# SamuelCancilla2/radar-point-cloud-tracking

Measured on AMD Instinct MI355X. Metric: Mpoints/s clustered+tracked, 1024-echo synthetic frames; 1/2/4/8-GPU scaling, higher is better.
Workload: dtype u8 echo / f32 geometry / f64 distance

## Files before the change

radar-point-cloud-tracking_amd/csrc/stdbscan.hip:

```cpp
#include <algorithm>
#include <cfloat>
#include <climits>
#include <cmath>
#include <cstdlib>
#include <cstring>
#include <mutex>
#include <vector>

#include "common.h"

#pragma clang fp contract(off)

namespace rpt {

namespace {

constexpr int kBlock = 256;

__device__ __forceinline__ uint32_t f2ord(float f) {
  uint32_t u = __float_as_uint(f);
  return (u & 0x80000000u) ? ~u : (u | 0x80000000u);
}
inline float ord2f(uint32_t u) {
  uint32_t v = (u & 0x80000000u) ? (u & 0x7fffffffu) : ~u;
// ... 173 lines not shown
    }
    sb[w].nonfinite_xyz = nonfin;
    sb[w].nonintegral_t = nonint;
    sb[w].n_finite_t = nfin;
    sb[w].t_descends = desc;
  }
  __syncthreads();
  if (threadIdx.x == 0) {
    for (int v = 1; v < kBlock / 64; ++v) {
      for (int k = 0; k < 4; ++k) {
        mn[k] = min(mn[k], sb[v].mn[k]);
        mx[k] = max(mx[k], sb[v].mx[k]);
      }
      nonfin |= sb[v].nonfinite_xyz;
      nonint |= sb[v].nonintegral_t;
      nfin += sb[v].n_finite_t;
      desc |= sb[v].t_descends;
    }
    for (int k = 0; k < 4; ++k) {
      out->mn[k] = mn[k];
      out->mx[k] = mx[k];
    }
    out->nonfinite_xyz = nonfin;
    out->nonintegral_t = nonint;
    out->n_finite_t = nfin;
    out->t_descends = desc;
  }
}

struct FastDiv {
  uint32_t m;
  int s;
  void init(uint32_t d) {
    int k = 0;
    while ((uint64_t(1) << k) < d) ++k;
    s = 31 + k;
    m = (uint32_t)(((uint64_t(1) << s) + d - 1) / d);
  }
  __device__ __forceinline__ uint32_t div(uint32_t n) const {
    return (uint32_t)(((uint64_t)n * m) >> s);
  }
};

struct Geom {
  double ox, oy, oz, ot;
  double cs;
  double ct;
  double inv_cs, inv_ct;
  int nx, ny, nz, nt;
  int64_t cells;
  double eps2;
  float epst;
  int min_samples;
  float e2lo, e2hi;
  int rt;
  int tfree;
  FastDiv fnx, fny, fnz, fslab;
  __device__ __forceinline__ void split(uint32_t k, int& x, int& y, int& z, int& s) const {
    const uint32_t r = fnx.div(k);
    x = (int)(k - r * (uint32_t)nx);
    const uint32_t r2 = fny.div(r);
    y = (int)(r - r2 * (uint32_t)ny);
    if (nz == 1) {
      z = 0;
      s = (int)r2;
    } else {
      const uint32_t r3 = fnz.div(r2);
      z = (int)(r2 - r3 * (uint32_t)nz);
      s = (int)r3;
    }
  }
  __device__ __forceinline__ int slab_of_key(int64_t k) const { return (int)fslab.div((uint32_t)k); }
};

__device__ __forceinline__ int cell_of(double v, double o, double inv, int n) {
  double q = floor((v - o) * inv);
  int c = (q < 0.0) ? 0 : (q >= (double)n ? n - 1 : (int)q);
  return c;
}
__device__ __forceinline__ int slab_of(float t, const Geom& g) {
  return cell_of((double)t, g.ot, g.inv_ct, g.nt);
}

template <int D>
__global__ __launch_bounds__(kBlock) void k_keys(const float* __restrict__ x,
                                                const float* __restrict__ y,
                                                const float* __restrict__ z, int64_t stride,
                                                const float* __restrict__ t, int64_t n, Geom g,
                                                uint32_t* __restrict__ keys,
                                                uint32_t* __restrict__ vals) {
  for (int64_t i = (int64_t)blockIdx.x * blockDim.x + threadIdx.x; i < n;
       i += (int64_t)gridDim.x * blockDim.x) {
    const float ti = t[i];
    uint32_t key;
    if (!isfinite(ti)) {
      key = (uint32_t)g.cells;
    } else {
      const int cx = cell_of((double)x[i * stride], g.ox, g.inv_cs, g.nx);
      const int cy = cell_of((double)y[i * stride], g.oy, g.inv_cs, g.ny);
      const int cz = (D == 3) ? cell_of((double)z[i * stride], g.oz, g.inv_cs, g.nz) : 0;
      const int s = slab_of(ti, g);
      key = (uint32_t)((((int64_t)s * g.nz + cz) * g.ny + cy) * g.nx + cx);
    }
    keys[i] = key;
    vals[i] = (uint32_t)i;
  }
}

template <int D>
__global__ __launch_bounds__(kBlock) void k_gather(const float* __restrict__ x,
                                                  const float* __restrict__ y,
                                                  const float* __restrict__ z, int64_t stride,
                                                  const float* __restrict__ t, int64_t n,
                                                  const uint32_t* __restrict__ skeys,
                                                  const uint32_t* __restrict__ svals,
                                                  float4* __restrict__ pts,
                                                  int32_t* __restrict__ sorig,
                                                  int32_t* __restrict__ skey,
                                                  int32_t* __restrict__ spos) {
  for (int64_t s = (int64_t)blockIdx.x * blockDim.x + threadIdx.x; s < n;
       s += (int64_t)gridDim.x * blockDim.x) {
    const int64_t i = svals[s];
    float4 p;
    p.x = x[i * stride];
    p.y = y[i * stride];
    p.w = t[i];
    p.z = (D == 3) ? z[i * stride] : p.w;
    pts[s] = p;
    sorig[s] = (int32_t)i;
    if (spos) spos[i] = (int32_t)s;
    skey[s] = (int32_t)skeys[s];
  }
}

__global__ __launch_bounds__(kBlock) void k_cell_runs(const int32_t* __restrict__ skey, int64_t n,
                                                     int32_t* __restrict__ cell_count,
                                                     int32_t* __restrict__ head) {
  for (int64_t s = (int64_t)blockIdx.x * blockDim.x + threadIdx.x; s < n;
       s += (int64_t)gridDim.x * blockDim.x) {
    const int32_t k = skey[s];
    const bool h = (s == 0) || skey[s - 1] != k;
    const bool t = (s == n - 1) || skey[s + 1] != k;
    if (h && t) {
      cell_count[k] = 1;
    } else {
      if (h) atomicAdd(cell_count + k, -(int32_t)s);
      if (t) atomicAdd(cell_count + k, (int32_t)(s + 1));
    }
    head[s] = h ? 1 : 0;
  }
}

__global__ __launch_bounds__(kBlock) void k_occ_list(const int32_t* __restrict__ skey, int64_t n,
                                                    const int32_t* __restrict__ pos,
                                                    int32_t* __restrict__ occ,
                                                    uint32_t* __restrict__ occ_bits) {
  for (int64_t s = (int64_t)blockIdx.x * blockDim.x + threadIdx.x; s < n;
       s += (int64_t)gridDim.x * blockDim.x)
    if (pos[s + 1] != pos[s]) {
      const int32_t c = skey[s];
      occ[pos[s]] = c;
      atomicOr(occ_bits + (c >> 5), 1u << (c & 31));
    }
}

constexpr int kBucketBlock = 1024;
// ... 2 lines not shown
constexpr int64_t kChunkPts = 16384;
static int slab_chunks_override() {
  static const int v = [] {
    const char* e = ab_env("RPT_SLAB_CHUNKS");
    return e ? std::atoi(e) : 0;
  }();
  return v;
}

static int ab_mode(const char* name) {
  const char* e = ab_env(name);
  const int v = e ? std::atoi(e) : 1;
  return (v == 0 || v == 2) ? v : 1;
}
static int cell_box_mixed() {
  static const int v = ab_mode("RPT_CELL_BOX_MIXED");
  return v;
}
static int union_snapshot() {
  static const int v = ab_mode("RPT_UNION_SNAP");
  return v;
}

static int label_core_orig() {
  static const int v = ab_mode("RPT_LABEL_ORIG");
  return v;
}

static bool cell_comp_enabled() {
  static const bool on = [] {
    const char* e = ab_env("RPT_CELL_COMP");
    return !(e && std::atoi(e) == 0);
  }();
  return on;
}

static bool chunk_scan_legacy() {
  static const bool v = [] {
    const char* e = ab_env("RPT_CHUNK_SCAN");
    return e && std::atoi(e) == 1;
  }();
  return v;
}

__global__ void k_slab_occ_base(const int32_t* __restrict__ pos, int P, int64_t nt,
                                int32_t* __restrict__ occ_base) {
  for (int64_t s = (int64_t)blockIdx.x * blockDim.x + threadIdx.x; s <= nt;
       s += (int64_t)gridDim.x * blockDim.x)
    occ_base[s] = pos[s * P];
}

__global__ void k_cell_start_end(int32_t* __restrict__ cell_start, int64_t cells) {
  if (threadIdx.x == 0) cell_start[cells + 1] = cell_start[cells];
}

__global__ void k_slab_lo(const float* __restrict__ t, int64_t n, Geom g,
                          int32_t* __restrict__ slab_lo, uint32_t* __restrict__ zero,
                          int64_t zwords) {
  for (int64_t i = (int64_t)blockIdx.x * blockDim.x + threadIdx.x; i < zwords;
       i += (int64_t)gridDim.x * blockDim.x)
    zero[i] = 0u;
  const int lane = threadIdx.x & 63;
  const int64_t wpb = blockDim.x / 64;
  for (int64_t s = (int64_t)blockIdx.x * wpb + threadIdx.x / 64; s <= g.nt;
       s += (int64_t)gridDim.x * wpb) {
    int64_t lo = 0, hi = n;
    while (lo < hi) {
      const int64_t step = (hi - lo + 63) / 64;
      const int64_t idx = lo + (int64_t)lane * step;
      const bool below = idx < hi && slab_of(t[idx < hi ? idx : lo], g) < s;
      const int c = __popcll(__ballot(below));
      if (c == 0) {
        hi = lo;
      } else {
        const int64_t nlo = lo + (int64_t)(c - 1) * step + 1;
        hi = min(hi, lo + (int64_t)c * step);
        lo = nlo;
      }
    }
    if (lane == 0) slab_lo[s] = (int32_t)(s == g.nt ? n : lo);
  }
}

__global__ __launch_bounds__(kBucketBlock) void k_slab_bucket(
    const float* __restrict__ x, const float* __restrict__ y, int64_t stride,
    const float* __restrict__ t, Geom g, const int32_t* __restrict__ slab_lo,
    float4* __restrict__ pts, int32_t* __restrict__ sorig, int32_t* __restrict__ skey,
    int32_t* __restrict__ spos, int32_t* __restrict__ cell_start, int32_t* __restrict__ occ_tmp,
    int32_t* __restrict__ slab_occ, uint32_t* __restrict__ occ_bits,
    unsigned long long* __restrict__ cmin_all = nullptr) {
  extern __shared__ int32_t hist[];
  __shared__ int32_t wsum[kBucketBlock / 64], wocc[kBucketBlock / 64];
  const int s = blockIdx.x;
  const int P = g.nx * g.ny;
  int32_t* mn = hist + P;
  const int lo = slab_lo[s], hi = slab_lo[s + 1];
  for (int c = threadIdx.x; c < P; c += kBucketBlock) {
    hist[c] = 0;
    if (cmin_all) mn[c] = INT_MAX;
  }
  __syncthreads();
  const int ln = threadIdx.x & 63;
  auto runs = [&](int c, bool v, int& rank, int& len, int& head) {
    const int up = __shfl_up(c, 1, 64), dn = __shfl_down(c, 1, 64);
    const uint64_t hm = __ballot(v && (ln == 0 || up != c));
    const uint64_t lm = __ballot(v && (ln == 63 || dn != c));
    const uint64_t below = (ln == 63) ? ~0ull : ((2ull << ln) - 1ull);
    head = 63 - __builtin_clzll((hm & below) | 1ull);
    const int last = ln + __builtin_ctzll((lm >> ln) | (1ull << (63 - ln)));
    rank = ln - head;
    len = last - head + 1;
  };
  auto cell_xy = [&](float px, float py) {
    return cell_of((double)py, g.oy, g.inv_cs, g.ny) * g.nx +
           cell_of((double)px, g.ox, g.inv_cs, g.nx);
  };
  for (int i0 = lo; i0 < hi; i0 += kBucketBlock * kBucketU) {
    float px[kBucketU], py[kBucketU];
#pragma unroll
    for (int u = 0; u < kBucketU; ++u) {
      const int i = min(i0 + u * kBucketBlock + (int)threadIdx.x, hi - 1);
      px[u] = x[(int64_t)i * stride];
      py[u] = y[(int64_t)i * stride];
    }
#pragma unroll
    for (int u = 0; u < kBucketU; ++u) {
      const int i = i0 + u * kBucketBlock + threadIdx.x;
      const bool v = i < hi;
      const int c = v ? cell_xy(px[u], py[u]) : -1;
      int rank, len, head;
      runs(c, v, rank, len, head);
      if (v && rank == 0) {
        atomicAdd(&hist[c], len);
        if (cmin_all) atomicMin(&mn[c], i);
      }
    }
  }
  __syncthreads();
  const int per = (P + kBucketBlock - 1) / kBucketBlock;
  const int c0 = threadIdx.x * per, c1 = min(c0 + per, P);
  int run = 0, orun = 0;
  for (int c = c0; c < c1; ++c) {
    const int h = hist[c];
    run += h;
    orun += (h > 0) ? 1 : 0;
  }
  const int lane = threadIdx.x & 63, w = threadIdx.x / 64;
  int incl = run, oincl = orun;
#pragma unroll
  for (int off = 1; off < 64; off <<= 1) {
    const int o = __shfl_up(incl, off, 64);
    const int oo = __shfl_up(oincl, off, 64);
    if (lane >= off) {
      incl += o;
      oincl += oo;
    }
  }
  if (lane == 63) {
    wsum[w] = incl;
    wocc[w] = oincl;
  }
  __syncthreads();
  int before = 0, obefore = 0, otot = 0;
  for (int v = 0; v < kBucketBlock / 64; ++v) {
    if (v < w) {
      before += wsum[v];
      obefore += wocc[v];
    }
    otot += wocc[v];
  }
  int acc = before + incl - run;
  int oacc = lo + obefore + oincl - orun;
  uint32_t word = 0xffffffffu, mask = 0u;
  for (int c = c0; c < c1; ++c) {
    const int h = hist[c];
    hist[c] = acc;
    cell_start[(int64_t)s * P + c] = lo + acc;
    acc += h;
    if (h > 0) {
      const int64_t key = (int64_t)s * P + c;
      occ_tmp[oacc++] = (int32_t)key;
      const uint32_t wd = (uint32_t)(key >> 5);
      if (wd != word) {
        if (mask) atomicOr(occ_bits + word, mask);
        word = wd;
        mask = 0u;
      }
      mask |= 1u << (key & 31);
    }
  }
  if (mask) atomicOr(occ_bits + word, mask);
  if (threadIdx.x == 0) slab_occ[s] = otot;
  __syncthreads();
  for (int i0 = lo; i0 < hi; i0 += kBucketBlock * kBucketU) {
    float px[kBucketU], py[kBucketU], pt[kBucketU];
#pragma unroll
    for (int u = 0; u < kBucketU; ++u) {
      const int i = min(i0 + u * kBucketBlock + (int)threadIdx.x, hi - 1);
      px[u] = x[(int64_t)i * stride];
      py[u] = y[(int64_t)i * stride];
      pt[u] = t[i];
    }
#pragma unroll
    for (int u = 0; u < kBucketU; ++u) {
      const int i = i0 + u * kBucketBlock + threadIdx.x;
      const bool v = i < hi;
      const int c = v ? cell_xy(px[u], py[u]) : -1;
      int rank, len, head;
      runs(c, v, rank, len, head);
      int base = (v && rank == 0) ? atomicAdd(&hist[c], len) : 0;
      base = __shfl(base, head, 64);
      if (v) {
        const int dst = lo + base + rank;
        pts[dst] = make_float4(px[u], py[u], pt[u], pt[u]);
        sorig[dst] = i;
        if (spos) spos[i] = dst;
        skey[dst] = s * P + c;
        if (cmin_all && mn[c] == i)
          cmin_all[(int64_t)s * P + c] = ((unsigned long long)(uint32_t)i << 32) | (uint32_t)dst;
      }
    }
  }
  if (s == g.nt - 1 && threadIdx.x == 0) {
    cell_start[g.cells] = hi;
    cell_start[g.cells + 1] = hi;
  }
}

__device__ __forceinline__ void slab_chunk(const int32_t* __restrict__ slab_lo, int s, int ch,
                                           int CH, int& lo, int& hi) {
  const int a = slab_lo[s], b = slab_lo[s + 1];
  const int64_t len = (int64_t)(b - a);
  lo = a + (int)(len * ch / CH);
  hi = a + (int)(len * (ch + 1) / CH);
}

__global__ __launch_bounds__(kBucketBlock) void k_slab_chunk_hist(
    const float* __restrict__ x, const float* __restrict__ y, int64_t stride, Geom g,
    const int32_t* __restrict__ slab_lo, int CH, int32_t* __restrict__ hist_g) {
  extern __shared__ int32_t hist[];
  const int s = blockIdx.x / CH, ch = blockIdx.x - s * CH;
  const int P = g.nx * g.ny;
  int lo, hi;
  slab_chunk(slab_lo, s, ch, CH, lo, hi);
  for (int c = threadIdx.x; c < P; c += kBucketBlock) hist[c] = 0;
  __syncthreads();
  for (int i0 = lo; i0 < hi; i0 += kBucketBlock * kBucketU) {
    float px[kBucketU], py[kBucketU];
#pragma unroll
    for (int u = 0; u < kBucketU; ++u) {
      const int i = min(i0 + u * kBucketBlock + (int)threadIdx.x, hi - 1);
      px[u] = x[(int64_t)i * stride];
      py[u] = y[(int64_t)i * stride];
    }
#pragma unroll
    for (int u = 0; u < kBucketU; ++u) {
      const int i = i0 + u * kBucketBlock + threadIdx.x;
      if (i < hi)
        atomicAdd(&hist[cell_of((double)py[u], g.oy, g.inv_cs, g.ny) * g.nx +
                        cell_of((double)px[u], g.ox, g.inv_cs, g.nx)], 1);
    }
  }
  __syncthreads();
  int32_t* out = hist_g + (int64_t)blockIdx.x * P;
  for (int c = threadIdx.x; c < P; c += kBucketBlock) out[c] = hist[c];
}

__global__ __launch_bounds__(kBucketBlock) void k_slab_chunk_scan(
    Geom g, const int32_t* __restrict__ slab_lo, int CH, int32_t* __restrict__ hist_g,
    int32_t* __restrict__ cell_start, int32_t* __restrict__ occ_tmp,
    int32_t* __restrict__ slab_occ, uint32_t* __restrict__ occ_bits) {
  __shared__ int32_t wsum[kBucketBlock / 64], wocc[kBucketBlock / 64];
  const int s = blockIdx.x;
  const int P = g.nx * g.ny;
  const int lo = slab_lo[s], hi = slab_lo[s + 1];
  int32_t* hs = hist_g + (int64_t)s * CH * P;
  const int per = (P + kBucketBlock - 1) / kBucketBlock;
  const int c0 = threadIdx.x * per, c1 = min(c0 + per, P);
  int run = 0, orun = 0;
  for (int c = c0; c < c1; ++c) {
    int h = 0;
    for (int ch = 0; ch < CH; ++ch) h += hs[(int64_t)ch * P + c];
    run += h;
    orun += (h > 0) ? 1 : 0;
  }
  const int lane = threadIdx.x & 63, w = threadIdx.x / 64;
  int incl = run, oincl = orun;
#pragma unroll
  for (int off = 1; off < 64; off <<= 1) {
    const int o = __shfl_up(incl, off, 64);
    const int oo = __shfl_up(oincl, off, 64);
    if (lane >= off) {
      incl += o;
      oincl += oo;
    }
  }
  if (lane == 63) {
// ... 8 lines not shown
      obefore += wocc[v];
    }
    otot += wocc[v];
  }
  int acc = before + incl - run;
  int oacc = lo + obefore + oincl - orun;
  uint32_t word = 0xffffffffu, mask = 0u;
  for (int c = c0; c < c1; ++c) {
    cell_start[(int64_t)s * P + c] = lo + acc;
    int h = 0;
    for (int ch = 0; ch < CH; ++ch) {
      const int k = hs[(int64_t)ch * P + c];
      hs[(int64_t)ch * P + c] = acc + h;
      h += k;
    }
    acc += h;
    if (h > 0) {
      const int64_t key = (int64_t)s * P + c;
      occ_tmp[oacc++] = (int32_t)key;
      const uint32_t wd = (uint32_t)(key >> 5);
      if (wd != word) {
        if (mask) atomicOr(occ_bits + word, mask);
        word = wd;
        mask = 0u;
      }
      mask |= 1u << (key & 31);
    }
  }
  if (mask) atomicOr(occ_bits + word, mask);
  if (threadIdx.x == 0) slab_occ[s] = otot;
  if (s == g.nt - 1 && threadIdx.x == 0) {
    cell_start[g.cells] = hi;
    cell_start[g.cells + 1] = hi;
  }
}

__global__ void k_chunk_totals(const int32_t* __restrict__ hist_g, int64_t cells, int P, int CH,
                               int32_t* __restrict__ cell_start) {
  for (int64_t k = (int64_t)blockIdx.x * blockDim.x + threadIdx.x; k < cells;
       k += (int64_t)gridDim.x * blockDim.x) {
    const int64_t s = k / P;
    const int32_t* h = hist_g + s * (int64_t)CH * P + (k - s * P);
    int t = 0;
    for (int ch = 0; ch < CH; ++ch) t += h[(int64_t)ch * P];
    cell_start[k] = t;
  }
}

__global__ void k_chunk_cursors(int32_t* __restrict__ hist_g, int64_t cells, int P, int CH,
                                const int32_t* __restrict__ cell_start,
                                const int32_t* __restrict__ slab_lo,
                                uint32_t* __restrict__ occ_bits, int32_t* __restrict__ occf) {
  const int lane = threadIdx.x & 63;
  for (int64_t k0 = ((int64_t)blockIdx.x * blockDim.x + threadIdx.x) & ~(int64_t)63; k0 < cells;
       k0 += (int64_t)gridDim.x * blockDim.x) {
    const int64_t k = k0 + lane;
    bool o = false;
    if (k < cells) {
      const int64_t s = k / P;
      int32_t* h = hist_g + s * (int64_t)CH * P + (k - s * P);
      int acc = cell_start[k] - slab_lo[s];
      const int first = acc;
      for (int ch = 0; ch < CH; ++ch) {
        const int v = h[(int64_t)ch * P];
        h[(int64_t)ch * P] = acc;
        acc += v;
      }
      o = acc > first;
      occf[k] = o ? 1 : 0;
    }
    const uint64_t m = __ballot(o);
    if (lane == 0) occ_bits[k0 >> 5] = (uint32_t)m;
    if (lane == 32) occ_bits[(k0 >> 5) + 1] = (uint32_t)(m >> 32);
  }
}

__global__ void k_occ_write(const int32_t* __restrict__ occf, const int32_t* __restrict__ pos,
                            int64_t cells, int32_t* __restrict__ occ) {
  for (int64_t k = (int64_t)blockIdx.x * blockDim.x + threadIdx.x; k < cells;
       k += (int64_t)gridDim.x * blockDim.x)
    if (occf[k]) occ[pos[k]] = (int32_t)k;
}

__global__ __launch_bounds__(kBucketBlock) void k_slab_chunk_scatter(
    const float* __restrict__ x, const float* __restrict__ y, int64_t stride,
    const float* __restrict__ t, Geom g, const int32_t* __restrict__ slab_lo, int CH,
    const int32_t* __restrict__ hist_g, float4* __restrict__ pts, int32_t* __restrict__ sorig,
    int32_t* __restrict__ skey, int32_t* __restrict__ spos) {
  extern __shared__ int32_t cur[];
  const int s = blockIdx.x / CH, ch = blockIdx.x - s * CH;
  const int P = g.nx * g.ny;
  int lo, hi;
  slab_chunk(slab_lo, s, ch, CH, lo, hi);
  const int base = slab_lo[s];
  const int32_t* hc = hist_g + (int64_t)blockIdx.x * P;
  for (int c = threadIdx.x; c < P; c += kBucketBlock) cur[c] = hc[c];
  __syncthreads();
  for (int i0 = lo; i0 < hi; i0 += kBucketBlock * kBucketU) {
    float px[kBucketU], py[kBucketU], pt[kBucketU];
#pragma unroll
    for (int u = 0; u < kBucketU; ++u) {
      const int i = min(i0 + u * kBucketBlock + (int)threadIdx.x, hi - 1);
      px[u] = x[(int64_t)i * stride];
      py[u] = y[(int64_t)i * stride];
      pt[u] = t[i];
    }
#pragma unroll
    for (int u = 0; u < kBucketU; ++u) {
      const int i = i0 + u * kBucketBlock + threadIdx.x;
      if (i < hi) {
        const int c = cell_of((double)py[u], g.oy, g.inv_cs, g.ny) * g.nx +
                      cell_of((double)px[u], g.ox, g.inv_cs, g.nx);
        const int dst = base + atomicAdd(&cur[c], 1);
        pts[dst] = make_float4(px[u], py[u], pt[u], pt[u]);
        sorig[dst] = i;
        if (spos) spos[i] = dst;
        skey[dst] = s * P + c;
      }
    }
  }
}

__global__ __launch_bounds__(kBlock) void k_occ_gather(const int32_t* __restrict__ occ_tmp,
                                                      const int32_t* __restrict__ slab_lo,
                                                      const int32_t* __restrict__ occ_base,
                                                      int32_t* __restrict__ occ) {
  const int s = blockIdx.x;
  const int b = occ_base[s], m = occ_base[s + 1] - b, lo = slab_lo[s];
  for (int j = threadIdx.x; j < m; j += blockDim.x) occ[b + j] = occ_tmp[lo + j];
}

__device__ __forceinline__ bool occupied(const uint32_t* __restrict__ bits, int64_t c) {
  return (bits[c >> 5] >> (c & 31)) & 1u;
}

static int wave_grid_cap() {
  static const int cap = [] {
    const char* e = ab_env("RPT_WAVE_GRID_CAP");
    const int v = e ? std::atoi(e) : 0;
    return v >= 8 ? v : 4096;
  }();
  return cap;
}
inline int wave_grid(int64_t max_items) {
  const int g = grid_for(max_items, kBlock / 64, wave_grid_cap());
  return (g + 7) & ~7;
}
constexpr int kDefaultUfFlags = 2;
inline int tile_grid(int64_t n) { return grid_for(n, kBlock * 16, 2048); }

__device__ __forceinline__ float wave_minf(float v) {
#pragma unroll
  for (int off = 32; off > 0; off >>= 1) v = fminf(v, __shfl_xor(v, off));
  return v;
}
__device__ __forceinline__ float wave_maxf(float v) {
#pragma unroll
  for (int off = 32; off > 0; off >>= 1) v = fmaxf(v, __shfl_xor(v, off));
  return v;
}
__device__ __forceinline__ int wave_sum(int v) {
  v = row_reduce<16>(v, OpAdd{});
  return __builtin_amdgcn_readlane(v, 0) + __builtin_amdgcn_readlane(v, 16) +
         __builtin_amdgcn_readlane(v, 32) + __builtin_amdgcn_readlane(v, 48);
}
__device__ __forceinline__ int wave_excl_sum(int v, int* total) {
  const int lane = threadIdx.x & 63;
  int incl = v;
#pragma unroll
  for (int off = 1; off < 64; off <<= 1) {
    const int o = __shfl_up(incl, off, 64);
    if (lane >= off) incl += o;
  }
  *total = __shfl(incl, 63, 64);
  return incl - v;
}
__device__ __forceinline__ int64_t wave_min64(int64_t v) {
#pragma unroll
  for (int off = 32; off > 0; off >>= 1) {
    const int64_t o = __shfl_xor(v, off);
    v = o < v ? o : v;
  }
  return v;
}

template <int D>
struct CellRec;
template <>
struct alignas(16) CellRec<2> {
  int b, e;
  float x0, x1, y0, y1, t0, t1;
};
template <>
struct alignas(16) CellRec<3> {
  int b, e;
  float x0, x1, y0, y1, z0, z1, t0, t1;
  int pad0, pad1;
};
template <int D>
__device__ __forceinline__ float4 rec_boxA(const CellRec<D>& r) {
  return make_float4(r.x0, r.x1, r.y0, r.y1);
}
__device__ __forceinline__ float4 rec_boxB(const CellRec<2>& r) {
  return make_float4(r.t0, r.t1, r.t0, r.t1);
}
__device__ __forceinline__ float4 rec_boxB(const CellRec<3>& r) {
  return make_float4(r.z0, r.z1, r.t0, r.t1);
}

constexpr int kCbLanes = 16;
template <int D>
__global__ __launch_bounds__(kBlock) void k_cell_box(const float4* __restrict__ pts,
                                                    const int32_t* __restrict__ cell_start,
                                                    const int32_t* __restrict__ occ,
                                                    const int32_t* __restrict__ n_occ, Geom g,
                                                    uint8_t* __restrict__ mutual,
                                                    CellRec<D>* __restrict__ crec,
                                                    unsigned long long* __restrict__ cmin =
                                                        nullptr,
                                                    const int32_t* __restrict__ sorig = nullptr) {
  constexpr int L = kCbLanes;
  const int j = threadIdx.x & (L - 1);
  const int64_t no = *n_occ;
  for (int64_t t = (int64_t)blockIdx.x * blockDim.x + threadIdx.x; t - j < no * L;
       t += (int64_t)gridDim.x * blockDim.x) {
    const int64_t q = t / L;
    const bool act = q < no;
    int c = 0, b = 0, e = 0;
    if (act) {
      c = occ[q];
      b = cell_start[c];
      e = cell_start[c + 1];
    }
    float x0 = FLT_MAX, x1 = -FLT_MAX, y0 = FLT_MAX, y1 = -FLT_MAX;
    float z0 = FLT_MAX, z1 = -FLT_MAX, t0 = FLT_MAX, t1 = -FLT_MAX;
    uint64_t mn = ~0ull;
    constexpr int kU = 8;
    for (int s0 = b + j; s0 < e; s0 += L * kU) {
      float4 pp[kU];
      uint32_t so[kU];
#pragma unroll
      for (int u = 0; u < kU; ++u) {
        const int s2 = s0 + L * u;
        const int sc = (s2 < e) ? s2 : s0;
        pp[u] = pts[sc];
        if (sorig) so[u] = (uint32_t)sorig[sc];
      }
#pragma unroll
      for (int u = 0; u < kU; ++u) {
        const float4 p = pp[u];
        x0 = fminf(x0, p.x); x1 = fmaxf(x1, p.x);
        y0 = fminf(y0, p.y); y1 = fmaxf(y1, p.y);
        z0 = fminf(z0, p.z); z1 = fmaxf(z1, p.z);
        t0 = fminf(t0, p.w); t1 = fmaxf(t1, p.w);
        if (sorig) {
          const int s2 = s0 + L * u;
          const uint64_t v = ((uint64_t)so[u] << 32) | (uint32_t)((s2 < e) ? s2 : s0);
          mn = v < mn ? v : mn;
        }
      }
    }
    if (sorig) mn = row_reduce<L>(mn, OpMin{});
    x0 = row_reduce<L>(x0, OpMin{}); x1 = row_reduce<L>(x1, OpMax{});
    y0 = row_reduce<L>(y0, OpMin{}); y1 = row_reduce<L>(y1, OpMax{});
    z0 = row_reduce<L>(z0, OpMin{}); z1 = row_reduce<L>(z1, OpMax{});
    t0 = row_reduce<L>(t0, OpMin{}); t1 = row_reduce<L>(t1, OpMax{});
    if (D != 3) {
      z0 = t0;
      z1 = t1;
    }
    if (act && j == 0) {
      CellRec<D> r{};
      r.b = b;
      r.e = e;
      r.x0 = x0;
      r.x1 = x1;
      r.y0 = y0;
      r.y1 = y1;
      if constexpr (D == 3) {
        r.z0 = z0;
        r.z1 = z1;
      }
      r.t0 = t0;
      r.t1 = t1;
      crec[c] = r;
      const double dx = (double)x1 - (double)x0;
      const double dy = (double)y1 - (double)y0;
      double d2 = dx * dx + dy * dy;
      if (D == 3) {
        const double dz = (double)z1 - (double)z0;
        d2 = d2 + dz * dz;
      }
      const float dt = t1 - t0;
      mutual[c] = (d2 <= g.eps2 && dt <= g.epst) ? 1 : 0;
      if (cmin) cmin[c] = sorig ? mn : ~0ull;
    }
  }
}

constexpr int kCbSmall = 4;
template <int D>
__device__ __forceinline__ void cell_box_store(int c, int b, int e, float x0, float x1, float y0,
                                               float y1, float z0, float z1, float t0, float t1,
                                               uint64_t mn, bool has_mn, const Geom& g,
                                               uint8_t* __restrict__ mutual,
                                               CellRec<D>* __restrict__ crec,
                                               unsigned long long* __restrict__ cmin) {
  CellRec<D> r{};
  r.b = b;
  r.e = e;
  r.x0 = x0;
  r.x1 = x1;
  r.y0 = y0;
  r.y1 = y1;
  if constexpr (D == 3) {
    r.z0 = z0;
    r.z1 = z1;
  }
  r.t0 = t0;
  r.t1 = t1;
  crec[c] = r;
  const double dx = (double)x1 - (double)x0;
  const double dy = (double)y1 - (double)y0;
  double d2 = dx * dx + dy * dy;
  if (D == 3) {
    const double dz = (double)z1 - (double)z0;
    d2 = d2 + dz * dz;
  }
  const float dt = t1 - t0;
  mutual[c] = (d2 <= g.eps2 && dt <= g.epst) ? 1 : 0;
  if (cmin) cmin[c] = has_mn ? mn : ~0ull;
}

template <int D>
__global__ __launch_bounds__(kBlock) void k_cell_box_mixed(const float4* __restrict__ pts,
                                                          const int32_t* __restrict__ cell_start,
                                                          const int32_t* __restrict__ occ,
                                                          const int32_t* __restrict__ n_occ,
                                                          Geom g, uint8_t* __restrict__ mutual,
                                                          CellRec<D>* __restrict__ crec,
                                                          unsigned long long* __restrict__ cmin =
                                                              nullptr,
                                                          const int32_t* __restrict__ sorig =
                                                              nullptr) {
  constexpr int L = kCbLanes;
  const int lane = threadIdx.x & 63;
  const int grp = lane / L, j = lane & (L - 1);
  const int64_t no = *n_occ;
  if (no == 0) return;
  const int64_t wpb = kBlock / 64;
  for (int64_t q0 = ((int64_t)blockIdx.x * wpb + threadIdx.x / 64) * 64; q0 < no;
       q0 += (int64_t)gridDim.x * wpb * 64) {
    const int64_t q = q0 + lane;
    const bool act = q < no;
    const int c = occ[act ? q : no - 1];
    const int b = cell_start[c], e = cell_start[c + 1];
    const bool small = act && e - b <= kCbSmall;
    {
      float4 pp[kCbSmall];
      uint32_t so[kCbSmall];
#pragma unroll
      for (int u = 0; u < kCbSmall; ++u) {
        const int sc = (b + u < e) ? b + u : b;
        pp[u] = pts[sc];
        if (sorig) so[u] = (uint32_t)sorig[sc];
      }
      float x0 = FLT_MAX, x1 = -FLT_MAX, y0 = FLT_MAX, y1 = -FLT_MAX;
      float z0 = FLT_MAX, z1 = -FLT_MAX, t0 = FLT_MAX, t1 = -FLT_MAX;
      uint64_t mn = ~0ull;
#pragma unroll
      for (int u = 0; u < kCbSmall; ++u) {
        const float4 p = pp[u];
        x0 = fminf(x0, p.x); x1 = fmaxf(x1, p.x);
        y0 = fminf(y0, p.y); y1 = fmaxf(y1, p.y);
        z0 = fminf(z0, p.z); z1 = fmaxf(z1, p.z);
        t0 = fminf(t0, p.w); t1 = fmaxf(t1, p.w);
        if (sorig) {
          const uint64_t v = ((uint64_t)so[u] << 32) | (uint32_t)((b + u < e) ? b + u : b);
          mn = v < mn ? v : mn;
        }
      }
      if (D != 3) {
        z0 = t0;
        z1 = t1;
      }
      if (small)
        cell_box_store<D>(c, b, e, x0, x1, y0, y1, z0, z1, t0, t1, mn, sorig != nullptr, g,
                          mutual, crec, cmin);
    }
    uint64_t big = __ballot(act && !small);
    while (big) {
      int pick = -1;
#pragma unroll
      for (int k = 0; k < 64 / L; ++k) {
        const int lk = big ? __ffsll((unsigned long long)big) - 1 : -1;
        if (grp == k) pick = lk;
        if (big) big &= big - 1;
      }
      const int src = pick < 0 ? 0 : pick;
      const int cc = __shfl(c, src), bb = __shfl(b, src), es = __shfl(e, src);
      const int ee = pick < 0 ? bb : es;
      float x0 = FLT_MAX, x1 = -FLT_MAX, y0 = FLT_MAX, y1 = -FLT_MAX;
      float z0 = FLT_MAX, z1 = -FLT_MAX, t0 = FLT_MAX, t1 = -FLT_MAX;
      uint64_t mn = ~0ull;
      constexpr int kU = 8;
      for (int s0 = bb + j; s0 < ee; s0 += L * kU) {
        float4 pp[kU];
        uint32_t so[kU];
#pragma unroll
        for (int u = 0; u < kU; ++u) {
          const int s2 = s0 + L * u;
          const int sc = (s2 < ee) ? s2 : s0;
          pp[u] = pts[sc];
          if (sorig) so[u] = (uint32_t)sorig[sc];
        }
#pragma unroll
        for (int u = 0; u < kU; ++u) {
          const float4 p = pp[u];
          x0 = fminf(x0, p.x); x1 = fmaxf(x1, p.x);
          y0 = fminf(y0, p.y); y1 = fmaxf(y1, p.y);
          z0 = fminf(z0, p.z); z1 = fmaxf(z1, p.z);
          t0 = fminf(t0, p.w); t1 = fmaxf(t1, p.w);
          if (sorig) {
            const int s2 = s0 + L * u;
            const uint64_t v = ((uint64_t)so[u] << 32) | (uint32_t)((s2 < ee) ? s2 : s0);
            mn = v < mn ? v : mn;
          }
        }
      }
      if (sorig) mn = row_reduce<L>(mn, OpMin{});
      x0 = row_reduce<L>(x0, OpMin{}); x1 = row_reduce<L>(x1, OpMax{});
      y0 = row_reduce<L>(y0, OpMin{}); y1 = row_reduce<L>(y1, OpMax{});
      z0 = row_reduce<L>(z0, OpMin{}); z1 = row_reduce<L>(z1, OpMax{});
      t0 = row_reduce<L>(t0, OpMin{}); t1 = row_reduce<L>(t1, OpMax{});
      if (D != 3) {
        z0 = t0;
        z1 = t1;
      }
      if (pick >= 0 && j == 0)
        cell_box_store<D>(cc, bb, ee, x0, x1, y0, y1, z0, z1, t0, t1, mn, sorig != nullptr, g,
                          mutual, crec, cmin);
    }
  }
}

template <int D>
__global__ __launch_bounds__(kBlock) void k_slab_range(const CellRec<D>* __restrict__ crec,
                                                      const int32_t* __restrict__ occ,
                                                      const int32_t* __restrict__ hpos,
                                                      const int32_t* __restrict__ cell_start,
                                                      int64_t cells_per_slab, int nt,
                                                      float2* __restrict__ slab_t,
                                                      const int32_t* __restrict__ occ_base) {
  const int s = blockIdx.x;
  if (s >= nt) return;
  const int q0 = occ_base ? occ_base[s] : hpos[cell_start[(int64_t)s * cells_per_slab]];
  const int q1 = occ_base ? occ_base[s + 1] : hpos[cell_start[(int64_t)(s + 1) * cells_per_slab]];
  float lo = FLT_MAX, hi = -FLT_MAX;
  for (int q = q0 + threadIdx.x; q < q1; q += blockDim.x) {
    const CellRec<D> r = crec[occ[q]];
    lo = fminf(lo, r.t0);
    hi = fmaxf(hi, r.t1);
  }
#pragma unroll
  for (int off = 32; off > 0; off >>= 1) {
    lo = fminf(lo, __shfl_xor(lo, off));
    hi = fmaxf(hi, __shfl_xor(hi, off));
  }
  __shared__ float slo[kBlock / 64], shi[kBlock / 64];
  if ((threadIdx.x & 63) == 0) {
    slo[threadIdx.x / 64] = lo;
    shi[threadIdx.x / 64] = hi;
  }
  __syncthreads();
  if (threadIdx.x == 0) {
    for (int w = 1; w < kBlock / 64; ++w) {
      lo = fminf(lo, slo[w]);
      hi = fmaxf(hi, shi[w]);
    }
    slab_t[s] = make_float2(lo, hi);
  }
}


template <int D>
__device__ __forceinline__ bool adjacent(const float4& a, const float4& b, const Geom& g) {
  const float dt = fabsf(a.w - b.w);
  const float fx = a.x - b.x, fy = a.y - b.y;
  float f2 = fx * fx + fy * fy;
  if (D == 3) {
    const float fz = a.z - b.z;
    f2 = f2 + fz * fz;
  }
  bool near = !(f2 <= g.e2lo) && !(f2 > g.e2hi);
  bool in = f2 <= g.e2lo;
  if (near) {
    const double dx = (double)a.x - (double)b.x;
    const double dy = (double)a.y - (double)b.y;
    double d2 = dx * dx + dy * dy;
    if (D == 3) {
      const double dz = (double)a.z - (double)b.z;
      d2 = d2 + dz * dz;
    }
    in = d2 <= g.eps2;
  }
  return in && (dt <= g.epst);
}

__device__ __forceinline__ void span_dist(float p, float lo, float hi, double& dmin,
                                          double& dmax) {
  const double dp = (double)p;
  dmin = (p < lo) ? ((double)lo - dp) : ((p > hi) ? (dp - (double)hi) : 0.0);
  dmax = fmax(fabs(dp - (double)lo), fabs(dp - (double)hi));
}

template <int D>
__device__ __forceinline__ int classify(const float4& p, const float4& A, const float4& B,
                                        const Geom& g) {
  const float tlo = B.z, thi = B.w;
  const float tmin = (p.w < tlo) ? (tlo - p.w) : ((p.w > thi) ? (p.w - thi) : 0.f);
  if (!(tmin <= g.epst)) return 0;
  const float tmax = fmaxf(fabsf(p.w - tlo), fabsf(p.w - thi));
  {
    auto fgap = [](float v, float lo, float hi) { return fmaxf(fmaxf(lo - v, v - hi), 0.f); };
    auto fspan = [](float v, float lo, float hi) { return fmaxf(fabsf(v - lo), fabsf(v - hi)); };
    const float gx = fgap(p.x, A.x, A.y), gy = fgap(p.y, A.z, A.w);
    const float sx = fspan(p.x, A.x, A.y), sy = fspan(p.y, A.z, A.w);
    float fmn = gx * gx + gy * gy, fmx = sx * sx + sy * sy;
    if (D == 3) {
      const float gz = fgap(p.z, B.x, B.y), sz = fspan(p.z, B.x, B.y);
      fmn = fmn + gz * gz;
      fmx = fmx + sz * sz;
    }
    if (fmn > g.e2hi) return 0;
    if (fmx <= g.e2lo) return (tmax <= g.epst) ? 1 : 2;
    if (fmn <= g.e2lo && fmx > g.e2hi) return 2;
  }
  double mnx, mxx, mny, mxy;
  span_dist(p.x, A.x, A.y, mnx, mxx);
  span_dist(p.y, A.z, A.w, mny, mxy);
  double dmin = mnx * mnx + mny * mny;
  double dmax = mxx * mxx + mxy * mxy;
  if (D == 3) {
    double mnz, mxz;
    span_dist(p.z, B.x, B.y, mnz, mxz);
    dmin = dmin + mnz * mnz;
    dmax = dmax + mxz * mxz;
  }
  if (!(dmin <= g.eps2)) return 0;
  return (dmax <= g.eps2 && tmax <= g.epst) ? 1 : 2;
}

template <int D, class F>
__device__ __forceinline__ void for_each_cell(const float4& p, int32_t key, const Geom& g,
                                              const int32_t* __restrict__ cell_start,
                                              const CellRec<D>* __restrict__ crec,
                                              const float2* __restrict__ slab_t, F&& f) {
  int cx, cy, cz, cs;
  g.split((uint32_t)key, cx, cy, cz, cs);
  const double tp = (double)p.w, et = (double)g.epst;
  int s0 = (int)fmax(floor((tp - et - g.ot) * g.inv_ct) - 1.0, 0.0);
  int s1 = (int)fmin(floor((tp + et - g.ot) * g.inv_ct) + 1.0, (double)(g.nt - 1));
  const int x0 = max(cx - 2, 0), x1 = min(cx + 2, g.nx - 1);
  const int y0 = max(cy - 2, 0), y1 = min(cy + 2, g.ny - 1);
  const int z0 = (D == 3) ? max(cz - 2, 0) : 0, z1 = (D == 3) ? min(cz + 2, g.nz - 1) : 0;
  (void)cs;
  for (int s = s0; s <= s1; ++s) {
    const float2 sr = slab_t[s];
    if (sr.x > sr.y) continue;
    const float smin = (p.w < sr.x) ? (sr.x - p.w) : ((p.w > sr.y) ? (p.w - sr.y) : 0.f);
    if (!(smin <= g.epst)) continue;
    for (int zz = z0; zz <= z1; ++zz) {
      for (int yy = y0; yy <= y1; ++yy) {
        const int64_t row = (((int64_t)s * g.nz + zz) * g.ny + yy) * g.nx;
        int b = cell_start[row + x0];
        for (int xx = x0; xx <= x1; ++xx) {
          const int e = cell_start[row + xx + 1];
          if (e > b) {
            const int64_t c = row + xx;
            const CellRec<D> cr = crec[c];
            const int cls = classify<D>(p, rec_boxA<D>(cr), rec_boxB(cr), g);
            if (cls != 0 && f(c, b, e, cls)) return;
          }
          b = e;
        }
      }
    }
  }
}

__device__ __forceinline__ int32_t rep_id(const int64_t* __restrict__ reps, int64_t nr, int64_t v) {
  int64_t lo = 0, hi = nr;
  while (lo < hi) {
    const int64_t m = (lo + hi) >> 1;
    if (reps[m] < v) lo = m + 1; else hi = m;
  }
  return (lo < nr && reps[lo] == v) ? (int32_t)lo : -2;
}

constexpr int kItems = 16;
struct AppendIndex {
  __device__ int32_t operator()(int64_t s) const { return (int32_t)s; }
};
template <class V = AppendIndex>
__device__ __forceinline__ void block_append_bits(int64_t tile0, uint32_t bits,
// ... 27 lines not shown
    const int o = __shfl_up(incl, off, 64);
    if (lane >= off) incl += o;
  }
  if (lane == 63) s_wsum[w] = incl;
  __syncthreads();
  int before = 0, total = 0;
#pragma unroll
  for (int v = 0; v < kBlock / 64; ++v) {
    const int t = s_wsum[v];
    before += (v < w) ? t : 0;
    total += t;
  }
  if (threadIdx.x == 0) s_base = total ? atomicAdd(counter, total) : 0;
  __syncthreads();
  int o = s_base + before + incl - c;
  while (bits) {
    const int k = __ffs(bits) - 1;
    bits &= bits - 1;
    list[o++] = value(tile0 + (int64_t)k * kBlock + threadIdx.x);
  }
  __syncthreads();
}

struct Window {
  int s0, x0, y0, z0;
  int nS;
  int total;
};

__device__ __forceinline__ bool slab_in_reach(const float2* __restrict__ slab_t, int s, float tlo,
                                              float thi, float epst) {
  const float2 sr = slab_t[s];
  if (sr.x > sr.y) return false;
  const float gap = (tlo > sr.y) ? (tlo - sr.y) : ((thi < sr.x) ? (sr.x - thi) : 0.f);
  return gap <= epst;
}

template <int D, bool SHRINK = true>
__device__ __forceinline__ Window make_window(int cx, int cy, int cz, float tlo, float thi,
                                              const Geom& g, const float2* __restrict__ slab_t,
                                              int s_min = 0) {
  constexpr int PER = (D == 3) ? 125 : 25;
  Window w;
  const double et = (double)g.epst;
  int s0, s1;
  if (g.rt >= 0) {
    s0 = max(slab_of(tlo, g) - g.rt, s_min);
    s1 = min(slab_of(thi, g) + g.rt, g.nt - 1);
  } else {
    s0 = (int)fmax(floor(((double)tlo - et - g.ot) * g.inv_ct) - 1.0, (double)s_min);
    s1 = (int)fmin(floor(((double)thi + et - g.ot) * g.inv_ct) + 1.0, (double)(g.nt - 1));
  }
  const int lane = threadIdx.x & 63;
  int lo = -1, hi = -1;
  if (!SHRINK) {
    lo = s0;
    hi = s1;
  }
  for (int c = s0; SHRINK && c <= s1; c += 64) {
    const bool ok = (c + lane <= s1) && slab_in_reach(slab_t, c + lane, tlo, thi, g.epst);
    const uint64_t m = __ballot(ok);
    if (m) {
      if (lo < 0) lo = c + __ffsll((unsigned long long)m) - 1;
      hi = c + 63 - __clzll((long long)m);
    }
  }
  if (lo < 0) {
    s0 = 0;
    s1 = -1;
  } else {
    s0 = lo;
    s1 = hi;
  }
  w.s0 = s0;
  w.nS = max(s1 - s0 + 1, 0);
  w.x0 = cx - 2;
  w.y0 = cy - 2;
  w.z0 = (D == 3) ? cz - 2 : 0;
  w.total = w.nS * PER;
  return w;
}

template <int D>
__device__ __forceinline__ void decode_key(int64_t key, const Geom& g, int& cx, int& cy, int& cz) {
  int cs;
  g.split((uint32_t)key, cx, cy, cz, cs);
  if (D != 3) cz = 0;
}

template <int D>
__device__ __forceinline__ int64_t window_cell(const Window& w, int q, const Geom& g,
                                               const float2* __restrict__ slab_t, float tlo,
                                               float thi) {
  constexpr int PER = (D == 3) ? 125 : 25;
  const int ss = q / PER;
  int r = q - ss * PER;
  int zz = 0;
  if (D == 3) {
    zz = r / 25;
    r -= zz * 25;
  }
  const int yy = r / 5, xx = r - yy * 5;
  const int x = w.x0 + xx, y = w.y0 + yy, z = w.z0 + zz;
  if (x < 0 || x >= g.nx || y < 0 || y >= g.ny || (D == 3 && (z < 0 || z >= g.nz))) return -1;
  const int sl = w.s0 + ss;
  return (((int64_t)sl * g.nz + z) * g.ny + y) * g.nx + x;
}

__device__ __forceinline__ float4 shfl_f4(const float4& v, int l) {
  return make_float4(__shfl(v.x, l), __shfl(v.y, l), __shfl(v.z, l), __shfl(v.w, l));
}

template <int D, bool SCREEN = false>
__device__ __forceinline__ int classify_cells(const float4& A1, const float4& B1,
                                              const float4& A2, const float4& B2,
                                              const Geom& g) {
  auto gap = [](float a0, float a1, float b0, float b1) -> float {
    return fmaxf(fmaxf(b0 - a1, a0 - b1), 0.f);
  };
  auto gapd = [](float a0, float a1, float b0, float b1) -> double {
    return (b0 > a1) ? ((double)b0 - (double)a1) : ((a0 > b1) ? ((double)a0 - (double)b1) : 0.0);
  };
  float tm = 0.f;
  if (!g.tfree) {
    const float tg = gap(A2.z, A2.w, B2.z, B2.w);
    if (!(tg <= g.epst)) return 0;
    tm = fmaxf(fabsf(B2.w - A2.z), fabsf(A2.w - B2.z));
  }
  if (D == 2 && SCREEN) {
    const float fx = gap(A1.x, A1.y, B1.x, B1.y), fy = gap(A1.z, A1.w, B1.z, B1.w);
    const float fmn = fx * fx + fy * fy;
    const float ux = fmaxf(fabsf(B1.y - A1.x), fabsf(A1.y - B1.x));
    const float uy = fmaxf(fabsf(B1.w - A1.z), fabsf(A1.w - B1.z));
    const float fmx = ux * ux + uy * uy;
    if (fmn > g.e2hi) return 0;
    if (fmx <= g.e2lo) return (tm <= g.epst) ? 1 : 2;
    if (fmn <= g.e2lo && fmx > g.e2hi) return 2;
  }
  const double gx = gapd(A1.x, A1.y, B1.x, B1.y), gy = gapd(A1.z, A1.w, B1.z, B1.w);
  double dmin = gx * gx + gy * gy;
  const double mx = fmax(fabs((double)B1.y - (double)A1.x), fabs((double)A1.y - (double)B1.x));
  const double my = fmax(fabs((double)B1.w - (double)A1.z), fabs((double)A1.w - (double)B1.z));
  double dmax = mx * mx + my * my;
  if (D == 3) {
    const double gz = gapd(A2.x, A2.y, B2.x, B2.y);
    dmin = dmin + gz * gz;
    const double mz = fmax(fabs((double)B2.y - (double)A2.x), fabs((double)A2.y - (double)B2.x));
    dmax = dmax + mz * mz;
  }
  if (!(dmin <= g.eps2)) return 0;
  return (dmax <= g.eps2 && tm <= g.epst) ? 1 : 2;
}

struct XcdRange {
  int64_t first, step, end;
};
__device__ __forceinline__ XcdRange xcd_items(int64_t n_items, bool remap) {
  const int64_t wpb = kBlock / 64, wave = threadIdx.x / 64;
  if (!remap || (gridDim.x & 7)) {
    return XcdRange{(int64_t)blockIdx.x * wpb + wave, (int64_t)gridDim.x * wpb, n_items};
  }
  const int64_t x = blockIdx.x & 7, lb = blockIdx.x >> 3, nbx = gridDim.x >> 3;
  const int64_t lo = n_items * x / 8, hi = n_items * (x + 1) / 8;
  return XcdRange{lo + lb * wpb + wave, nbx * wpb, hi};
}

constexpr int kR = 4;
static_assert(kR >= 2, "the union passes' candidate masks cover two 64-position rounds");
constexpr uint32_t kPmaskFull = 0x80000000u;
static bool cell_roots_enabled() {
  static const bool on = [] {
    const char* e = ab_env("RPT_CELL_ROOTS");
    return !(e && std::atoi(e) == 0);
  }();
  return on;
}

__global__ __launch_bounds__(kBlock) void k_core_cell_fast(const int32_t* __restrict__ occ,
                                                          const int32_t* __restrict__ n_occ,
                                                          Geom g,
                                                          const int32_t* __restrict__ cell_start,
                                                          const uint8_t* __restrict__ mutual,
                                                          int32_t* __restrict__ cflag,
                                                          int32_t* __restrict__ queue,
                                                          int32_t* __restrict__ n_queue) {
  const int need = g.min_samples;
  const int64_t no = *n_occ;
  for (int64_t tile = (int64_t)blockIdx.x * kBlock * kItems; tile < no;
       tile += (int64_t)gridDim.x * kBlock * kItems) {
    block_append(
        tile, no,
        [&](int64_t q) -> bool {
// ... 442 lines not shown
  const int need = g.min_samples;
  const XcdRange xr = xcd_items(*n_slow, true);
  for (int64_t q = xr.first; q < xr.end; q += xr.step) {
    const int s = slow[q];
    const int32_t key = slowk ? slowk[q] : skey[s];
    const float4 p = pts[s];
    int cx, cy, cz;
    decode_key<D>(key, g, cx, cy, cz);
    Window w;
    if (slowk && g.rt >= 0) {
      const int cs = g.slab_of_key(key);
      w.s0 = max(cs - g.rt, 0);
      w.nS = max(min(cs + g.rt, g.nt - 1) - w.s0 + 1, 0);
      w.x0 = cx - 2;
      w.y0 = cy - 2;
      w.z0 = (D == 3) ? cz - 2 : 0;
      w.total = w.nS * ((D == 3) ? 125 : 25);
    } else {
      w = make_window<D, false>(cx, cy, cz, p.w, p.w, g, slab_t);
    }
    int cnt = 0;
    for (int base = 0; base < w.total && cnt < need; base += 64 * KR) {
      int64_t c[KR];
      uint32_t wb[KR];
#pragma unroll
      for (int r = 0; r < KR; ++r) {
        const int qq = base + r * 64 + lane;
        c[r] = (qq < w.total) ? window_cell<D>(w, qq, g, slab_t, p.w, p.w) : -1;
      }
#pragma unroll
      for (int r = 0; r < KR; ++r) wb[r] = (c[r] >= 0) ? occ_bits[c[r] >> 5] : 0u;
      int b[KR], e[KR], cls[KR];
#pragma unroll
      for (int r = 0; r < KR; ++r) {
        b[r] = e[r] = cls[r] = 0;
        if (c[r] >= 0 && ((wb[r] >> (c[r] & 31)) & 1u)) {
          const CellRec<D> cr = crec[c[r]];
          b[r] = cr.b;
          e[r] = cr.e;
          cls[r] = classify<D>(p, rec_boxA<D>(cr), rec_boxB(cr), g);
        }
      }
      int add = 0, may = 0;
#pragma unroll
      for (int r = 0; r < KR; ++r) {
        add += (cls[r] == 1) ? e[r] - b[r] : 0;
        may += (cls[r] == 2) ? e[r] - b[r] : 0;
      }
      cnt += wave_sum(add);
      const bool last = base + 64 * KR >= w.total;
      if (last && cnt + wave_sum(may) < need) break;
#pragma unroll
      for (int r = 0; r < KR; ++r) {
        uint64_t pm = __ballot(cls[r] == 2);
        while (pm && cnt < need) {
          const int l = __ffsll((unsigned long long)pm) - 1;
          pm &= pm - 1;
          const int bb = __shfl(b[r], l), ee = __shfl(e[r], l);
          for (int j0 = bb; j0 < ee && cnt < need; j0 += 64) {
            const int j = j0 + lane;
            const bool a = (j < ee) && adjacent<D>(p, pts[j], g);
            cnt += __popcll(__ballot(a));
          }
        }
      }
    }
    if (lane == 0) {
      core[s] = (cnt >= need) ? 1 : 0;
      if (cmin && cnt >= need && (int64_t)key < g.cells)
        atomicMin(cmin + key, ((unsigned long long)(uint32_t)sorig[s] << 32) | (uint32_t)s);
    }
  }
}

__device__ __forceinline__ int mask_pos_key(int pos, const Geom& g, int R, int W, uint32_t mg,
                                            int cx, int cy, int cs) {
  const int P = pos / 5, dx = pos - 5 * P;
  const int k = min((int)(((uint32_t)P * mg) >> 16), 4);
  const int si = P - k * W;
  const int s2 = cs + si - R;
  const int y = cy + cw_row(k) - 2;
  return (s2 * g.ny + y) * g.nx + (cx - 2 + dx);
}
__global__ __launch_bounds__(kBlock, 8) void k_core_slow_masked(
    const float4* __restrict__ pts, Geom g, int R, const CellRec<2>* __restrict__ crec,
    const int32_t* __restrict__ occ, const int32_t* __restrict__ slow,
    const int32_t* __restrict__ slowq, const int32_t* __restrict__ n_slow,
    const uint4* __restrict__ pmask, const int32_t* __restrict__ clo, uint8_t* __restrict__ core,
    const int32_t* __restrict__ sorig, unsigned long long* __restrict__ cmin) {
  const int lane = threadIdx.x & 63;
  const int need = g.min_samples;
  const int W = 2 * R + 1;
  const uint32_t mg = (65535u + (uint32_t)W) / (uint32_t)W;
  const XcdRange xr = xcd_items(*n_slow, true);
  for (int64_t q = xr.first; q < xr.end; q += xr.step) {
    const int s = slow[q];
    const int32_t cq = slowq[q];
    const float4 p = pts[s];
    const int32_t key = occ[cq];
    const uint4 m = pmask[cq];
    int cnt = clo[cq];
    int cx, cy, cz, cs;
    g.split((uint32_t)key, cx, cy, cz, cs);
    const uint32_t w0 = lane < 32 ? m.x : m.y;
    const uint32_t w1 = lane < 32 ? m.z : m.w;
    const bool h0 = (w0 >> (lane & 31)) & 1u, h1 = (w1 >> (lane & 31)) & 1u;
    const int k0 = h0 ? mask_pos_key(lane, g, R, W, mg, cx, cy, cs) : key;
    const int k1 = h1 ? mask_pos_key(lane + 64, g, R, W, mg, cx, cy, cs) : key;
    const CellRec<2> c0 = crec[k0], c1 = crec[k1];
    const int cl0 = h0 ? classify<2>(p, rec_boxA<2>(c0), rec_boxB(c0), g) : 0;
    const int cl1 = h1 ? classify<2>(p, rec_boxA<2>(c1), rec_boxB(c1), g) : 0;
    int add = (cl0 == 1 ? c0.e - c0.b : 0) + (cl1 == 1 ? c1.e - c1.b : 0);
    int may = (cl0 == 2 ? c0.e - c0.b : 0) + (cl1 == 2 ? c1.e - c1.b : 0);
    cnt += wave_sum(add);
    if (cnt < need && cnt + wave_sum(may) >= need) {
#pragma unroll
      for (int r = 0; r < 2; ++r) {
        const int cl = r ? cl1 : cl0;
        const int bq = r ? c1.b : c0.b, eq = r ? c1.e : c0.e;
        uint64_t pm = __ballot(cl == 2);
        while (pm && cnt < need) {
          const int l = __ffsll((unsigned long long)pm) - 1;
          pm &= pm - 1;
          const int bb = __shfl(bq, l), ee = __shfl(eq, l);
          for (int j0 = bb; j0 < ee && cnt < need; j0 += 64) {
            const int jj = j0 + lane;
            const bool a = (jj < ee) && adjacent<2>(p, pts[jj], g);
            cnt += __popcll(__ballot(a));
          }
        }
      }
    }
    if (lane == 0) {
      core[s] = (cnt >= need) ? 1 : 0;
      if (cmin && cnt >= need)
        atomicMin(cmin + key, ((unsigned long long)(uint32_t)sorig[s] << 32) | (uint32_t)s);
    }
  }
}

__global__ __launch_bounds__(kBlock) void k_cell_min_pair(const int32_t* __restrict__ skey,
                                                         const uint8_t* __restrict__ core,
                                                         const int32_t* __restrict__ sorig,
                                                         int64_t n, int64_t cells,
                                                         unsigned long long* __restrict__ cmin) {
  const int lane = threadIdx.x & 63;
  for (int64_t s0 = (int64_t)blockIdx.x * blockDim.x; s0 < n;
       s0 += (int64_t)gridDim.x * blockDim.x) {
    const int64_t s = s0 + threadIdx.x;
    const int key = (s < n) ? skey[s] : -1;
    uint64_t v = (s < n && core[s] && (int64_t)key < cells)
                     ? (((uint64_t)(uint32_t)sorig[s] << 32) | (uint32_t)s)
                     : ~0ull;
#pragma unroll
    for (int off = 1; off < 64; off <<= 1) {
      const uint32_t olo = (uint32_t)__shfl_up((int)(uint32_t)v, off, 64);
      const uint32_t ohi = (uint32_t)__shfl_up((int)(uint32_t)(v >> 32), off, 64);
      const int ok = __shfl_up(key, off, 64);
      if (lane >= off && ok == key) v = min(v, ((uint64_t)ohi << 32) | olo);
    }
    const int next = __shfl_down(key, 1, 64);
    if ((lane == 63 || next != key) && key >= 0 && v != ~0ull)
      atomicMin(cmin + key, (unsigned long long)v);
  }
}

__global__ __launch_bounds__(kBlock) void k_init_occ_cells(const int32_t* __restrict__ occ,
                                                          const int32_t* __restrict__ n_occ,
                                                          int64_t cells,
                                                          int32_t* __restrict__ rep,
                                                          unsigned long long* __restrict__ cmin,
                                                          int32_t* __restrict__ zero_counter =
                                                              nullptr,
                                                          int32_t* __restrict__ zero_counter2 =
                                                              nullptr) {
  if (blockIdx.x == 0 && threadIdx.x == 0) {
    if (zero_counter) *zero_counter = 0;
    if (zero_counter2) *zero_counter2 = 0;
  }
  const int64_t m = *n_occ;
  for (int64_t q = (int64_t)blockIdx.x * blockDim.x + threadIdx.x; q < m;
       q += (int64_t)gridDim.x * blockDim.x) {
    const int32_t c = occ[q];
    if ((int64_t)c < cells) {
      rep[c] = -1;
      if (cmin) cmin[c] = ~0ull;
    }
  }
}

constexpr int kPU = 8;
__global__ __launch_bounds__(kBlock) void k_parent_init_pair(
    int32_t* __restrict__ parent, int64_t n, const uint8_t* __restrict__ core,
    const int32_t* __restrict__ skey, const uint8_t* __restrict__ mutual,
    const unsigned long long* __restrict__ cmin, int64_t cells, int32_t* __restrict__ rep) {
  for (int64_t tile = (int64_t)blockIdx.x * kBlock * kPU; tile < n;
       tile += (int64_t)gridDim.x * kBlock * kPU) {
    int32_t k[kPU];
    uint32_t c[kPU];
#pragma unroll
    for (int u = 0; u < kPU; ++u) {
      const int64_t s = min(tile + (int64_t)u * kBlock + threadIdx.x, n - 1);
      k[u] = skey[s];
      c[u] = core[s];
    }
    bool q[kPU];
    unsigned long long m[kPU];
    uint32_t mu[kPU];
#pragma unroll
    for (int u = 0; u < kPU; ++u) {
// ... 367 lines not shown
          int64_t cb[kR];
          uint32_t wb[kR];
          int rb[kR], cls[kR];
#pragma unroll
          for (int k = 0; k < kR; ++k) {
            const int qq = base + k * W + hl;
            cb[k] = (qq < w.total) ? window_cell<2>(w, qq, g, slab_t, A2.z, A2.w) : -1;
            if (cb[k] <= (int64_t)ca) cb[k] = -1;
          }
#pragma unroll
          for (int k = 0; k < kR; ++k) wb[k] = (cb[k] >= 0) ? occ_bits[cb[k] >> 5] : 0u;
#pragma unroll
          for (int k = 0; k < kR; ++k) {
            rb[k] = -1;
            cls[k] = 0;
            if (cb[k] >= 0 && ((wb[k] >> (cb[k] & 31)) & 1u)) {
              const CellRec<2> cr = crec[cb[k]];
              const int r = rep[cb[k]];
              const uint8_t m = mutual[cb[k]];
              if (r >= 0 && m) {
                rb[k] = r;
                cls[k] = classify_cells<2>(A1, rec_boxA<2>(cr), A2, rec_boxB(cr), g);
              }
            }
          }
          if (pmask && base == 0) {
            uint32_t wd[kR];
#pragma unroll
            for (int k = 0; k < kR; ++k) wd[k] = hbal(cls[k] == 2);
            static_assert(kR == 4, "the 128-bit pmask holds 4 x 32 window positions");
            if (hl == 0)
              pmask[q] = (w.total < 128)
                             ? make_uint4(wd[0], wd[1], wd[2], wd[3] & ~kPmaskFull)
                             : make_uint4(0u, 0u, 0u, kPmaskFull);
            any_und = w.total >= 128 || (wd[0] | wd[1] | wd[2] | wd[3]) != 0u;
          }
          const int rA = uf_find(parent, ra, halve);
#pragma unroll
          for (int k = 0; k < kR; ++k) {
            const int rt = (cls[k] == 1) ? uf_find(parent, rb[k], halve) : -1;
            bool pend = rt >= 0 && rt != rA;
            bool mine = false;
            uint32_t pm = hbal(pend);
            while (pm) {
              const int l = h0 + __ffs(pm) - 1;
              const int v = __shfl(rt, l);
              mine = mine || (lane == l);
              pend = pend && (rt != v);
              pm = hbal(pend);
            }
            if (mine) uf_unite(parent, sorig, rA, rt, halve);
          }
        }
      }
      const bool u0 = __shfl((int)any_und, 0) != 0, u1 = __shfl((int)any_und, 32) != 0;
      if (u0) lmask |= 1ull << l0;
      if (u1 && l1 >= 0) lmask |= 1ull << l1;
    }
    if (plist) s_pl.push(lmask, ql, lane, plist, pcount);
  }
  if ((plist || nm_list) && block_last_wave(&s_done, lane)) {
    if (plist) s_pl.flush(lane, plist, pcount);
    if (nm_list) s_nm.flush(lane, nm_list, nm_count);
  }
}

__global__ __launch_bounds__(kBlock) void k_cell_root_snapshot(const int32_t* __restrict__ occ,
                                                              const int32_t* __restrict__ n_occ,
                                                              const int32_t* __restrict__ rep,
                                                              int32_t* __restrict__ parent,
                                                              int64_t cells, int uf_flags,
                                                              int32_t* __restrict__ croot) {
  const bool halve = !(uf_flags & 1);
  const int64_t no = *n_occ;
  for (int64_t q = (int64_t)blockIdx.x * blockDim.x + threadIdx.x; q < no;
       q += (int64_t)gridDim.x * blockDim.x) {
    const int c = occ[q];
    if ((int64_t)c >= cells) continue;
    const int r = rep[c];
    croot[c] = r >= 0 ? uf_find(parent, r, halve) : -1;
  }
}

__global__ __launch_bounds__(kBlock) void k_union_listed(const float4* __restrict__ pts, Geom g,
                                                        const int32_t* __restrict__ occ,
                                                        const CellRec<2>* __restrict__ crec,
                                                        const uint32_t* __restrict__ occ_bits,
                                                        const float2* __restrict__ slab_t,
                                                        const uint8_t* __restrict__ core,
                                                        const int32_t* __restrict__ rep,
                                                        const uint8_t* __restrict__ mutual,
                                                        const int32_t* __restrict__ sorig,
                                                        int32_t* __restrict__ parent, int uf_flags,
                                                        const uint4* __restrict__ pmask,
                                                        const int32_t* __restrict__ plist,
                                                        const int32_t* __restrict__ pcount,
                                                        const int32_t* __restrict__ croot,
                                                        int32_t* __restrict__ lstat = nullptr) {
  const int lane = threadIdx.x & 63;
  const bool halve = !(uf_flags & 1);
  const XcdRange xr = xcd_items(*pcount, false);
  if (xr.first >= xr.end) return;
  auto list_at = [&](int64_t ii) { return plist[ii < xr.end ? ii : xr.end - 1]; };
  int ca = occ[list_at(xr.first)];
  uint4 pm = pmask[list_at(xr.first)];
  int qn = list_at(xr.first + xr.step);
  for (int64_t i = xr.first; i < xr.end; i += xr.step) {
    const int ra = rep[ca];
    const int sra = croot ? croot[ca] : -1;
    const CellRec<2> ra_rec = crec[ca];
    const int can = occ[qn];
    const uint4 pmn = pmask[qn];
    const int qnn = list_at(i + 2 * xr.step);
    const int ba = ra_rec.b, ea = ra_rec.e;
    const float4 A1 = rec_boxA<2>(ra_rec), A2 = rec_boxB(ra_rec);
    int cx, cy, cz;
    decode_key<2>(ca, g, cx, cy, cz);
    const int sa = g.slab_of_key(ca);
    const Window w = make_window<2, false>(cx, cy, cz, A2.z, A2.w, g, slab_t, sa);
    auto settle = [&](int rb, int bb, int eb) {
      const int rbr = rb >= 0 ? uf_find(parent, rb, halve) : -1;
      const bool cand = rb >= 0 && uf_find(parent, ra, halve) != rbr;
      uint64_t cm = __ballot(cand);
#ifdef RPT_AB
      if (lstat) {
        const int nb = __popcll(__ballot(rb >= 0));
        if (lane == 0) {
          atomicAdd(&lstat[0], nb);
          atomicAdd(&lstat[1], __popcll(cm));
        }
      }
#endif
      while (cm) {
        const int l = __ffsll((unsigned long long)cm) - 1;
        cm &= cm - 1;
        const int rbl = __shfl(rb, l);
        const int ebl = __shfl(eb, l);
        const int bbl = __shfl(bb, l);
        if (uf_find(parent, ra, halve) == uf_find(parent, rbl, halve)) continue;
#ifdef RPT_AB
        if (lstat && lane == 0) atomicAdd(&lstat[2], 1);
#endif
        bool hit = false;
        for (int jb0 = bbl; jb0 < ebl && !hit; jb0 += 64) {
          const int jb = jb0 + lane;
          float4 pb = make_float4(0.f, 0.f, 0.f, 0.f);
          bool cb_ok = false;
          if (jb < ebl && core[jb]) {
            pb = pts[jb];
            cb_ok = classify<2>(pb, A1, A2, g) != 0;
          }
          const uint64_t bm = __ballot(cb_ok);
          for (int ja0 = ba; bm && ja0 < ea && !hit; ja0 += 64) {
            const int ja = ja0 + lane;
            const bool va = (ja < ea) && core[ja];
            const float4 pa = va ? pts[ja] : make_float4(0.f, 0.f, 0.f, 0.f);
            bool adj = false;
            uint64_t rest = bm;
            while (rest) {
              const int lb = __ffsll((unsigned long long)rest) - 1;
              rest &= rest - 1;
              const float4 pq = shfl_f4(pb, lb);
              adj = adj || (va && adjacent<2>(pq, pa, g));
            }
            hit = __ballot(adj) != 0;
          }
        }
        if (hit) {
#ifdef RPT_AB
          if (lstat && lane == 0) atomicAdd(&lstat[3], 1);
#endif
          if (lane == 0) uf_unite(parent, sorig, ra, rbl, halve);
          const int rr = __shfl(rbr, l);
          cm &= ~__ballot(rbr == rr);
        }
      }
    };
    if (!(pm.w & kPmaskFull)) {
      int rb[2], ebv[2], bbv[2];
#pragma unroll
      for (int k = 0; k < 2; ++k) {
        rb[k] = -1;
        ebv[k] = bbv[k] = 0;
        const uint32_t word = k == 0 ? (lane < 32 ? pm.x : pm.y) : (lane < 32 ? pm.z : pm.w);
        if ((word >> (lane & 31)) & 1u) {
          const int64_t c = window_cell<2>(w, k * 64 + lane, g, slab_t, A2.z, A2.w);
          if (!croot || croot[c] != sra) {
            const CellRec<2> cr = crec[c];
            rb[k] = rep[c];
            ebv[k] = cr.e;
            bbv[k] = cr.b;
          }
        }
      }
      settle(rb[0], bbv[0], ebv[0]);
      settle(rb[1], bbv[1], ebv[1]);
    } else {
      for (int base = 0; base < w.total; base += 64) {
        const int qq = base + lane;
        int64_t c = (qq < w.total) ? window_cell<2>(w, qq, g, slab_t, A2.z, A2.w) : -1;
        if (c <= (int64_t)ca || !((occ_bits[c >> 5] >> (c & 31)) & 1u)) c = -1;
        int rb = -1, bb = 0, eb = 0;
        if (c >= 0) {
          const CellRec<2> cr = crec[c];
          const int r = rep[c];
          if (r >= 0 && mutual[c] &&
              classify_cells<2>(A1, rec_boxA<2>(cr), A2, rec_boxB(cr), g) == 2) {
            rb = r;
            bb = cr.b;
            eb = cr.e;
          }
        }
        settle(rb, bb, eb);
      }
    }
    ca = can;
    pm = pmn;
    qn = qnn;
  }
}

template <int D>
__device__ __forceinline__ void union_point(int si, int32_t key, const float4* __restrict__ pts,
                                            Geom g, const int32_t* __restrict__ cell_start,
                                            const CellRec<D>* __restrict__ crec,
                                            const float2* __restrict__ slab_t,
                                            const uint8_t* __restrict__ core,
                                            const int32_t* __restrict__ rep,
                                            const uint8_t* __restrict__ mutual,
                                            const int32_t* __restrict__ sorig,
                                            int32_t* __restrict__ parent) {
  const float4 p = pts[si];
  for_each_cell<D>(p, key, g, cell_start, crec, slab_t,
                   [&](int64_t c, int b, int e, int cls) -> bool {
                     const int r = rep[c];
                     if (r < 0) return false;
                     if (mutual[c]) {
                       if (cls == 1) {
                         uf_unite(parent, sorig, si, r);
                         return false;
                       }
                       if (uf_find(parent, si) == uf_find(parent, r)) return false;
                       for (int j = b; j < e; ++j) {
                         if (core[j] && adjacent<D>(p, pts[j], g)) {
                           uf_unite(parent, sorig, si, j);
                           break;
// ... 282 lines not shown
    const int root = uf_find(parent, r);
    const int32_t k = sorig[root];
    cell_key[c] = k;
    if (root == r) atomicOr(min_bits + (k >> 5), 1u << (k & 31));
  }
}

struct AppendSpos {
  const int32_t* spos;
  __device__ int32_t operator()(int64_t i) const { return spos[i]; }
};
template <bool ORIG>
__global__ __launch_bounds__(kBlock) void k_label_core_cells(
    const int32_t* __restrict__ skey, const uint8_t* __restrict__ core,
    const int32_t* __restrict__ perm, int64_t n, int64_t cells,
    const int32_t* __restrict__ cell_key, MinRank cid, int32_t* __restrict__ labels,
    int32_t* __restrict__ nc_list, int32_t* __restrict__ nc_count,
    const int32_t* __restrict__ guard, int32_t* __restrict__ n_clusters) {
  if (blockIdx.x == 0 && threadIdx.x == 0 && *guard != 0) *n_clusters = -1;
  const int64_t T = (n + (int64_t)kBlock * kPU - 1) / ((int64_t)kBlock * kPU);
  const bool xm = (gridDim.x & 7) == 0;
  const int64_t xg = blockIdx.x & 7, nbx = gridDim.x >> 3;
  const int64_t t_lo = xm ? T * xg / 8 : blockIdx.x, t_hi = xm ? T * (xg + 1) / 8 : T;
  const int64_t t_step = xm ? nbx : gridDim.x;
  for (int64_t ti = t_lo + (xm ? (int64_t)(blockIdx.x >> 3) : 0); ti < t_hi; ti += t_step) {
    const int64_t tile = ti * kBlock * kPU;
    int32_t pv[kPU], k[kPU];
    uint32_t c[kPU];
    if (ORIG) {
#pragma unroll
      for (int u = 0; u < kPU; ++u)
        pv[u] = __builtin_nontemporal_load(perm + min(tile + (int64_t)u * kBlock + threadIdx.x,
                                                       n - 1));
#pragma unroll
      for (int u = 0; u < kPU; ++u) {
        k[u] = skey[pv[u]];
        c[u] = core[pv[u]];
      }
    } else {
#pragma unroll
      for (int u = 0; u < kPU; ++u) {
        const int64_t s = min(tile + (int64_t)u * kBlock + threadIdx.x, n - 1);
        k[u] = skey[s];
        c[u] = core[s];
        pv[u] = perm[s];
      }
    }
    int32_t own[kPU];
    uint32_t inb = 0, cb = 0;
#pragma unroll
    for (int u = 0; u < kPU; ++u) {
      const bool in = tile + (int64_t)u * kBlock + threadIdx.x < n;
      const bool q = in && c[u] != 0u && k[u] >= 0 && (int64_t)k[u] < cells;
      inb |= in ? (1u << u) : 0u;
      cb |= (in && c[u] != 0u) ? (1u << u) : 0u;
      const int32_t v = cell_key[q ? k[u] : 0];
      own[u] = (q && v != INT_MAX) ? v : -1;
    }
    uint32_t w[kPU];
    int32_t pr[kPU];
#pragma unroll
    for (int u = 0; u < kPU; ++u) {
      const int32_t m = own[u] >= 0 ? own[u] : 0;
      w[u] = cid.bits[m >> 5];
      pr[u] = cid.pref[m >> 5];
    }
#pragma unroll
    for (int u = 0; u < kPU; ++u) {
      if (own[u] >= 0) {
        const int32_t lab = pr[u] + __popc(w[u] & ((1u << (own[u] & 31)) - 1u));
        if (ORIG)
          labels[tile + (int64_t)u * kBlock + threadIdx.x] = lab;
        else
          labels[pv[u]] = lab;
      }
    }
    if (ORIG)
      block_append_bits(tile, inb & ~cb, nc_list, nc_count, AppendSpos{perm});
    else
      block_append_bits(tile, inb & ~cb, nc_list, nc_count);
  }
}

template <int D, bool GLOBAL, int W = 64, bool ALLMUT = false>
__global__ __launch_bounds__(kBlock, 6) void k_label(const float4* __restrict__ pts,
                                                 const int32_t* __restrict__ skey, Geom g,
                                                 const CellRec<D>* __restrict__ crec,
                                                 const uint32_t* __restrict__ occ_bits,
                                                 const float2* __restrict__ slab_t,
                                                 const int32_t* __restrict__ key_of,
                                                 const int32_t* __restrict__ cell_key,
                                                 const uint8_t* __restrict__ mutual,
                                                 const int32_t* __restrict__ sorig,
                                                 MinRank cid,
                                                 const int32_t* __restrict__ nc_list,
                                                 const int32_t* __restrict__ nc_count,
                                                 int32_t* __restrict__ labels,
                                                 int32_t* __restrict__ kstat = nullptr,
                                                 const uint8_t* __restrict__ core_of = nullptr) {
  static_assert(!ALLMUT || (D == 2 && !GLOBAL), "all-mutual grids are 2-D, local runs");
  static_assert(W == 32 || W == 64, "a point per wave or per half-wave");
  constexpr int P = 64 / W;
  const int lane = threadIdx.x & 63;
  const int hl = lane & (W - 1);
  const int h0 = lane - hl;
  const int shift = (W == 64) ? 0 : h0;
  auto gbal = [&](bool v) -> uint64_t {
    const uint64_t b = __ballot(v);
    return (W == 64) ? b : ((b >> shift) & 0xffffffffull);
  };
  auto gmin = [&](int v) -> int {
    v = row_reduce<16>(v, OpMin{});
    v = min(v, __shfl_xor(v, 16));
    if (W == 64) v = min(v, __shfl_xor(v, 32));
    return v;
  };
  const int64_t nc = *nc_count;
  const XcdRange xr = xcd_items((nc + P - 1) / P, true);
  for (int64_t qp = xr.first; qp < xr.end; qp += xr.step) {
    const int64_t q = qp * P + (lane / W);
    if (q >= nc) continue;
    const int s = nc_list[q];
    const int32_t key = skey[s];
    int best = INT_MAX;
#ifdef RPT_AB
    bool st_core = false, st_search = false;
#endif
    if ((int64_t)key < g.cells) {
      const float4 p = pts[s];
      int cx, cy, cz;
      decode_key<D>(key, g, cx, cy, cz);
      const Window w = make_window<D, false>(cx, cy, cz, p.w, p.w, g, slab_t);
      for (int base = 0; base < w.total; base += W * kR) {
        int64_t c[kR];
        int ck[kR], cb[kR], ce[kR], cls[kR], mu[kR];
#pragma unroll
        for (int k = 0; k < kR; ++k) {
          const int qq = base + k * W + hl;
          c[k] = (qq < w.total) ? window_cell<D>(w, qq, g, slab_t, p.w, p.w) : -1;
        }
#pragma unroll
        for (int k = 0; k < kR; ++k) ck[k] = (c[k] >= 0) ? cell_key[c[k]] : INT_MAX;
        int v = INT_MAX;
#pragma unroll
        for (int k = 0; k < kR; ++k) {
          cb[k] = ce[k] = cls[k] = mu[k] = 0;
          if (ck[k] != INT_MAX) {
            const CellRec<D> cr = crec[c[k]];
            cb[k] = cr.b;
            ce[k] = cr.e;
            mu[k] = ALLMUT ? 1 : mutual[c[k]];
            cls[k] = classify<D>(p, rec_boxA<D>(cr), rec_boxB(cr), g);
            if (cls[k] == 1) v = min(v, ck[k]);
          }
        }
        best = min(best, gmin(v));
#ifdef RPT_AB
        {
          bool anyc = false;
#pragma unroll
          for (int k = 0; k < kR; ++k) anyc = anyc || ck[k] != INT_MAX;
          st_core = st_core || gbal(anyc) != 0;
        }
#endif
        uint32_t pend = 0;
#pragma unroll
        for (int k = 0; k < kR; ++k) pend |= (cls[k] == 2) ? (1u << k) : 0u;
        while (true) {
          int mine = INT_MAX, mk = -1;
#pragma unroll
          for (int k = 0; k < kR; ++k)
            if (((pend >> k) & 1u) && ck[k] < best && ck[k] < mine) {
              mine = ck[k];
              mk = k;
            }
          const int mm = gmin(mine);
          if (mm == INT_MAX) break;
#ifdef RPT_AB
          st_search = true;
#endif
          const uint64_t at = gbal(mine == mm);
          const int l = h0 + __ffsll((unsigned long long)at) - 1;
          const int kl = __shfl(mk, l);
          int bsel = 0, esel = 0, msel = 0;
#pragma unroll
          for (int k = 0; k < kR; ++k)
            if (k == kl) {
              bsel = cb[k];
              esel = ce[k];
              msel = mu[k];
            }
          if (lane == l) pend &= ~(1u << kl);
          const int bl = __shfl(bsel, l), el = __shfl(esel, l);
          if (ALLMUT || __shfl(msel, l)) {
            bool hit = false;
            for (int j0 = bl; j0 < el && !hit; j0 += 2 * W) {
              const int j = j0 + hl, j2 = j + W;
              const bool v1 = j < el, v2 = j2 < el;
              int k1, k2;
              if (ALLMUT) {
                k1 = (v1 && core_of[j]) ? 0 : -1;
                k2 = (v2 && core_of[j2]) ? 0 : -1;
              } else {
                k1 = v1 ? key_of[j] : -1;
                k2 = v2 ? key_of[j2] : -1;
              }
              const float4 p1 = v1 ? pts[j] : p, p2 = v2 ? pts[j2] : p;
              hit = gbal((k1 >= 0 && adjacent<D>(p, p1, g)) ||
                         (k2 >= 0 && adjacent<D>(p, p2, g))) != 0;
            }
            if (hit) best = mm;
          } else {
            int lb = INT_MAX;
            for (int j0 = bl; j0 < el; j0 += 2 * W) {
              const int j = j0 + hl, j2 = j + W;
              const bool v1 = j < el, v2 = j2 < el;
              const int m1 = v1 ? key_of[j] : -1, m2 = v2 ? key_of[j2] : -1;
              const float4 p1 = v1 ? pts[j] : p, p2 = v2 ? pts[j2] : p;
              if (m1 >= 0 && m1 < best && m1 < lb && adjacent<D>(p, p1, g)) lb = m1;
              if (m2 >= 0 && m2 < best && m2 < lb && adjacent<D>(p, p2, g)) lb = m2;
            }
            best = min(best, gmin(lb));
          }
        }
      }
    }
    if (hl == 0) {
      int32_t out = -1;
      if (best != INT_MAX) out = GLOBAL ? best : cid[best];
      labels[sorig[s]] = out;
#ifdef RPT_AB
      if (kstat) {
        atomicAdd(&kstat[0], 1);
        if (st_core) atomicAdd(&kstat[1], 1);
        if (st_search) atomicAdd(&kstat[2], 1);
        if (best != INT_MAX) atomicAdd(&kstat[3], 1);
      }
#endif
    }
  }
}

#ifdef RPT_AB
#include "stdbscan_ab.inc"
#endif

__global__ __launch_bounds__(kBlock) void k_isolated_labels(int32_t* labels, int64_t n,
                                                           int singletons) {
  for (int64_t i = (int64_t)blockIdx.x * blockDim.x + threadIdx.x; i < n;
       i += (int64_t)gridDim.x * blockDim.x)
    labels[i] = singletons ? (int32_t)i : -1;
}


__global__ void k_core_to_orig(const uint8_t* __restrict__ core, const int32_t* __restrict__ sorig,
                               int64_t n, uint8_t* __restrict__ out) {
  for (int64_t s = (int64_t)blockIdx.x * blockDim.x + threadIdx.x; s < n;
       s += (int64_t)gridDim.x * blockDim.x)
    out[sorig[s]] = core[s];
}
__global__ void k_core_from_orig(const uint8_t* __restrict__ in, const int32_t* __restrict__ sorig,
                                 int64_t n, uint8_t* __restrict__ core) {
  for (int64_t s = (int64_t)blockIdx.x * blockDim.x + threadIdx.x; s < n;
       s += (int64_t)gridDim.x * blockDim.x)
    core[s] = in[sorig[s]] ? 1 : 0;
}
__global__ void k_comp_out(int32_t* parent, const uint8_t* __restrict__ core,
                           const int32_t* __restrict__ sorig, int64_t n,
                           int32_t* __restrict__ comp, const int32_t* __restrict__ skey,
                           const int32_t* __restrict__ cell_root, int64_t cells) {
  for (int64_t s = (int64_t)blockIdx.x * blockDim.x + threadIdx.x; s < n;
       s += (int64_t)gridDim.x * blockDim.x) {
    int32_t out = -1;
    if (core[s]) {
      const int32_t key = skey[s];
      const int32_t cr = ((int64_t)key < cells) ? cell_root[key] : -1;
      out = sorig[cr >= 0 ? cr : uf_find(parent, (int)s)];
    }
    comp[sorig[s]] = out;
  }
}
__global__ void k_comp_out_edges(int32_t* parent, const uint8_t* __restrict__ core,
                                 const int32_t* __restrict__ sorig, int64_t n,
                                 int32_t* __restrict__ comp, const int32_t* __restrict__ skey,
                                 const int32_t* __restrict__ cell_root, int64_t cells,
                                 int64_t lo_end, int64_t hi_begin) {
  for (int64_t s = (int64_t)blockIdx.x * blockDim.x + threadIdx.x; s < n;
       s += (int64_t)gridDim.x * blockDim.x) {
    const int32_t i = sorig[s];
    if (i >= lo_end && i < hi_begin) continue;
    int32_t out = -1;
    if (core[s]) {
      const int32_t key = skey[s];
      const int32_t cr = (cell_root && (int64_t)key < cells) ? cell_root[key] : -1;
      out = sorig[cr >= 0 ? cr : uf_find(parent, (int)s)];
    }
    comp[i] = out;
  }
}
__global__ __launch_bounds__(kBlock) void k_ccmin_global(int32_t* parent,
                                                        const uint8_t* __restrict__ core,
                                                        int64_t n,
                                                        const int32_t* __restrict__ sorig,
// ... 462 lines not shown
  }
  int uf_compress = -1;
  uint32_t* min_bits = nullptr;
  int32_t* min_pref = nullptr;
  int64_t min_words() const { return n / 32 + 1; }
  int32_t* n_clusters_ptr() const { return min_pref + min_words(); }
  int32_t cluster_ids(hipStream_t st, int32_t* cell_key, int32_t* zero = nullptr);
  int32_t* cell_root = nullptr;
  int uf_flags = -1;
  int k5_legacy = -1;
  int k5_fill = 0;
  int k5_fused = -1;
  bool bucket_allmin = false;
  void k5_env() {
    if (k5_legacy < 0) {
      const char* e = ab_env("RPT_K5_MODE");
      k5_legacy = e ? std::atoi(e) : 0;
      k5_legacy = (k5_legacy == 0) ? 1 : 0;
      k5_fill = (e && std::atoi(e) == 2) ? 1 : 0;
    }
    if (k5_tiles < 0) {
      const char* e = ab_env("RPT_K5_TILES");
      k5_tiles = (e && std::atoi(e) == 1) ? 1 : 0;
    }
    if (k5_fused < 0) {
      const char* e = ab_env("RPT_K5_FUSED");
      k5_fused = (e && std::atoi(e) == 0) ? 0 : 1;
    }
  }
  int k5_mask_ = -1;
  bool k5_mask() {
    if (k5_mask_ < 0) {
      const char* e = ab_env("RPT_K5_MASK");
      k5_mask_ = (e && std::atoi(e) == 0) ? 0 : 1;
    }
    return k5_mask_ == 1;
  }
  bool k5_fused_path() {
    k5_env();
    return oct_ok() && k5_legacy && k5_fused && !k5_tiles;
  }
  int k5_tiles = -1;
  int k7_tiles = -1;
  int32_t* rowq = nullptr;
  int32_t* rowcnt = nullptr;
  bool rowq_ok = false;
  int tile_by = 0, tile_nbands = 0, tile_R = 0;
  bool use_label_tiles() {
    if (k7_tiles < 0) {
      const char* e = ab_env("RPT_K7_TILES");
      k7_tiles = (e && std::atoi(e) == 1) ? 1 : 0;
    }
    return k7_tiles && rowq_ok && dim == 2 && g.nz == 1;
  }
  unsigned tile_grid_blocks() const {
    return (unsigned)((((int64_t)g.nt * tile_nbands + 1) + 7) & ~(int64_t)7);
  }
  double slab_reach() const {
    return integral_t ? std::ceil(std::floor((double)g.epst) / g.ct)
                      : std::ceil((double)g.epst / g.ct) + 1.0;
  }
  bool oct_ok() const { return dim == 2 && g.nz == 1 && slab_reach() <= (double)kCwMaxR; }
  int k7_w = -1;
  int label_w() {
    if (k7_w < 0) {
      const char* e = ab_env("RPT_K7_W");
      k7_w = (e && std::atoi(e) == 64) ? 64 : 32;
    }
    return k7_w;
  }
  int bucket_mode = -1;
  template <int D>
  const CellRec<D>* rec() const {
    return static_cast<const CellRec<D>*>(crec);
  }
  int32_t* slab = nullptr;
  bool spos_on = false;
  bool dense_slabs = false;
  int32_t* cell_min = nullptr;
  uint8_t* fok = nullptr;
  bool integral_t = false;
  bool all_mutual = false;
  bool cell_comp = false;
  int64_t* stmp = nullptr;
  Timer tm;

  template <int D>
  int32_t build_t(const float* x, const float* y, const float* z, int64_t stride, const float* t,
                  double eps_space, double eps_time, hipStream_t st);
  const void* given_bounds = nullptr;
  int32_t build(const float* x, const float* y, const float* z, int64_t stride, const float* t,
                int64_t n_, double eps_space, double eps_time, int32_t ms, bool timing,
                hipStream_t st);
  int32_t core_pass(hipStream_t st);
  int32_t union_pass(hipStream_t st, bool fused = false);
  int32_t labels_local(int32_t* labels, rpt_stdbscan_stats* stats, hipStream_t st);
  bool defer = false;
  int32_t fill_stats(int32_t n_clusters, rpt_stdbscan_stats* stats);
  int32_t labels_global(const int64_t* rep_orig, const int64_t* reps, int64_t nr,
                        int32_t* labels, hipStream_t st, const int64_t* nr_dev = nullptr);
  int32_t frames_pass(int32_t min_frames, hipStream_t st);
  int32_t labels_fifo(int32_t* labels, rpt_stdbscan_stats* stats, hipStream_t st);
};

template <int D>
int32_t DbscanState::build_t(const float* x, const float* y, const float* z, int64_t stride,
                             const float* t, double eps_space, double eps_time, hipStream_t st) {
  const int gb = grid_for(n, kBlock, 2048);
  const int nbb = grid_for(n, kBlock, 1024);
  {
    Budget bb;
    bb.add<Bounds>(1);
    bb.add<Bounds>(nbb);
    RPT_TRY(arena.reserve(bb.bytes, st));
  }
  Bounds* d_b = arena.carve_n<Bounds>(1);
  Bounds* d_part = arena.carve_n<Bounds>(nbb);
  Bounds hb;
  if (given_bounds) {
    std::memcpy(&hb, given_bounds, sizeof(Bounds));
  } else {
    hipLaunchKernelGGL(k_bounds<D>, dim3(nbb), dim3(kBlock), 0, st, x, y, z, stride, t, n,
                       d_part, (const int64_t*)nullptr);
    hipLaunchKernelGGL(k_bounds_final, dim3(1), dim3(kBlock), 0, st, d_part, nbb, d_b);
    RPT_CHECK_LAUNCH();
    RPT_HIP(hipMemcpyAsync(&hb, d_b, sizeof(Bounds), hipMemcpyDeviceToHost, st));
    RPT_TRY(wait_stream(st));
  }
  tm.mark();
  if (hb.nonfinite_xyz) {
    set_error("Input contains NaN or infinity in coordinates");
    return RPT_ENONFINITE;
  }
  const float epst = (float)eps_time;
  g = Geom{};
  g.eps2 = eps_space * eps_space;
  g.epst = epst;
  static const bool screen_on = [] {
    const char* e = ab_env("RPT_F32_SCREEN");
    return !(e && e[0] == '0');
  }();
  const bool screen = screen_on && g.eps2 >= 1e-20 && g.eps2 <= 1e30;
  g.e2lo = screen ? (float)(g.eps2 * (1.0 - 1e-5)) : -1.0f;
  g.e2hi = screen ? (float)(g.eps2 * (1.0 + 1e-5)) : INFINITY;
  g.min_samples = min_samples;
  double lo[4], hi[4];
  for (int k = 0; k < 4; ++k) {
    lo[k] = (double)ord2f(hb.mn[k]);
    hi[k] = (double)ord2f(hb.mx[k]);
  }
  if (hb.n_finite_t == 0) lo[3] = hi[3] = 0.0;
  integral_t = !hb.nonintegral_t;
  const double margin = 1.0 + 1.0 / 1048576.0;
  static const double side_f = [] {
    const char* e = ab_env("RPT_CELL_SIDE");
    const double v = e ? std::atof(e) : 0.0;
    return (v >= 0.5 && v <= 0.7) ? v : 0.7;
  }();
  const double sf = (D == 2) ? side_f : 0.5;
  double cs = (eps_space > 0.0 ? eps_space * sf : 1.0) * margin;
  double ct = !hb.nonintegral_t ? 1.0 : (epst > 0.f ? (double)epst : 1.0) * margin;
  const int64_t cmax = std::min<int64_t>(std::max<int64_t>(int64_t(1) << 22, 4 * n),
                                         int64_t(1) << 30);
  auto dims = [&](double ext, double side) -> int64_t {
    const double q = floor(ext / side) + 1.0;
    return q > 1e9 ? (int64_t)1e9 : (int64_t)q;
// ... 39 lines not shown
  Budget bud;
  bud.add<Bounds>(1);
  for (int k = 0; k < 4; ++k) bud.add<uint32_t>(n);
  bud.add<int64_t>(radix_tmp_elems(n));
  bud.add<float4>(n);
  bud.add<int32_t>(n);
  bud.add<int32_t>(n);
  bud.add<int32_t>(C1 + 1);
  bud.add<int64_t>(scan_tmp_elems(C1 + 1) + scan_tmp_elems(n + 1));
  bud.add<uint8_t>(C1);
  bud.add<int32_t>(C1);
  bud.add<float2>(nt);
  bud.add<uint8_t>(n);
  bud.add<int32_t>(n);
  bud.add<int32_t>(n);
  bud.add<int32_t>(n + 1);
  bud.add<int32_t>(n + 1);
  bud.add<int32_t>(n);
  bud.add<uint8_t>(C1);
  bud.add<int32_t>(C1);
  bud.add<int32_t>(C1);
  bud.add<uint64_t>(C1);
  bud.add<uint32_t>(n / 32 + 1);
  bud.add<int32_t>(n / 32 + 2);
  bud.add<int32_t>(n + 1);
  bud.add<int32_t>(n + 1);
  bud.add<CellRec<D>>(C1);
  bud.add<uint32_t>(C1 / 32 + 2);
  bud.add<int32_t>(nt + 1);
  bud.add<int32_t>(nt + 1);
  bud.add<int32_t>(nt + 1);
  bud.add<int32_t>((size_t)(ny * nz * nt) + 1);
  bud.add<int32_t>((size_t)(ny * nz * nt) + 1);
  RPT_TRY(arena.reserve(bud.bytes, st));
  (void)arena.carve_n<Bounds>(1);
  uint32_t* keys = arena.carve_n<uint32_t>(n);
  uint32_t* vals = arena.carve_n<uint32_t>(n);
  uint32_t* keys_alt = arena.carve_n<uint32_t>(n);
  uint32_t* vals_alt = arena.carve_n<uint32_t>(n);
  pmask = reinterpret_cast<uint4*>(keys);
  int64_t* rtmp = arena.carve_n<int64_t>(radix_tmp_elems(n));
  pts = arena.carve_n<float4>(n);
  sorig = arena.carve_n<int32_t>(n);
  skey = arena.carve_n<int32_t>(n);
  cell_start = arena.carve_n<int32_t>(C1 + 1);
  stmp = arena.carve_n<int64_t>(scan_tmp_elems(C1 + 1) + scan_tmp_elems(n + 1));
  mutual = arena.carve_n<uint8_t>(C1);
  rep = arena.carve_n<int32_t>(C1);
  slab_t = arena.carve_n<float2>(nt);
  core = arena.carve_n<uint8_t>(n);
  parent = arena.carve_n<int32_t>(n);
  ccmin = arena.carve_n<int32_t>(n);
  cid = arena.carve_n<int32_t>(n + 1);
  nc_list = arena.carve_n<int32_t>(n + 1);
  slab = arena.carve_n<int32_t>(n);
  fok = arena.carve_n<uint8_t>(C1);
  cell_min = arena.carve_n<int32_t>(C1);
  cell_root = arena.carve_n<int32_t>(C1);
  cell_min_pair = arena.carve_n<uint64_t>(C1);
  min_bits = arena.carve_n<uint32_t>(n / 32 + 1);
  min_pref = arena.carve_n<int32_t>(n / 32 + 2);
  occ = arena.carve_n<int32_t>(n + 1);
  hpos = arena.carve_n<int32_t>(n + 1);
  CellRec<D>* cr = arena.carve_n<CellRec<D>>(C1);
  crec = cr;
  occ_bits = arena.carve_n<uint32_t>(C1 / 32 + 2);
  int32_t* slab_lo = arena.carve_n<int32_t>(nt + 1);
  int32_t* slab_occ = arena.carve_n<int32_t>(nt + 1);
  int32_t* occ_base = arena.carve_n<int32_t>(nt + 1);
  rowq = arena.carve_n<int32_t>((size_t)(ny * nz * nt) + 1);
  rowcnt = arena.carve_n<int32_t>((size_t)(ny * nz * nt) + 1);
  rowq_ok = false;
  if (!slab_lo || !rowcnt) {
    set_error("internal: scratch carve overflow");
    return RPT_ENOMEM;
  }
  if (bucket_mode < 0) {
    const char* e = ab_env("RPT_K4_BUCKET");
    bucket_mode = (e && std::atoi(e) == 0) ? 0 : 1;
  }
  bucket_allmin = false;
  const bool bucket = bucket_mode && D == 2 && hb.n_finite_t == n && !hb.t_descends &&
                      (int64_t)nx * ny <= kBucketCells && nt < (int64_t(1) << 31);
  if (bucket) {
    hipLaunchKernelGGL(k_slab_lo, dim3(grid_for(64 * (nt + 1), kBlock, 4096)), dim3(kBlock), 0,
                       st, t, n, g, slab_lo, occ_bits, (int64_t)(C1 / 32 + 2));
    const size_t hist_bytes = sizeof(int32_t) * (size_t)nx * ny;
    const int64_t avg = n / std::max<int64_t>(nt, 1);
    dense_slabs = avg > 8 * kChunkPts;
    spos_on = label_core_orig() == 2 || (label_core_orig() == 1 && dense_slabs);
    int32_t* spos_w = spos_on ? slab : nullptr;
    int64_t ch = avg > 8 * kChunkPts ? (avg + kChunkPts - 1) / kChunkPts : 1;
    ch = std::max<int64_t>(ch, (512 + nt - 1) / std::max<int64_t>(nt, 1));
    int CH = (int)std::min<int64_t>(ch, 64);
    while (CH > 1 && (int64_t)nt * CH * nx * ny > 4 * n) --CH;
    if (slab_chunks_override() > 0) CH = slab_chunks_override();
    const bool coalesced_scan = CH >= 8 && (int64_t)nt * CH * nx * ny <= 4 * n &&
                                !chunk_scan_legacy();
    if (CH > 1 && (int64_t)nt * CH * nx * ny <= 4 * n) {
      int32_t* hist_g = reinterpret_cast<int32_t*>(keys);
      RPT_HIP(hipFuncSetAttribute((const void*)k_slab_chunk_hist,
                                  hipFuncAttributeMaxDynamicSharedMemorySize, (int)hist_bytes));
      RPT_HIP(hipFuncSetAttribute((const void*)k_slab_chunk_scatter,
                                  hipFuncAttributeMaxDynamicSharedMemorySize, (int)hist_bytes));
      hipLaunchKernelGGL(k_slab_chunk_hist, dim3((unsigned)(nt * CH)), dim3(kBucketBlock),
                         hist_bytes, st, x, y, stride, g, slab_lo, CH, hist_g);
      if (!coalesced_scan) {
        hipLaunchKernelGGL(k_slab_chunk_scan, dim3((unsigned)nt), dim3(kBucketBlock), 0, st, g,
                           slab_lo, CH, hist_g, cell_start, hpos, slab_occ, occ_bits);
      } else {
        const int64_t cells = (int64_t)nt * nx * ny;
        const int P = (int)(nx * ny);
        const int gc = grid_for(cells, kBlock, 8192);
        hipLaunchKernelGGL(k_chunk_totals, dim3(gc), dim3(kBlock), 0, st, hist_g, cells, P, CH,
                           cell_start);
        RPT_TRY(exclusive_scan_total_i32(cell_start, cell_start, cells, st));
        hipLaunchKernelGGL(k_chunk_cursors, dim3(gc), dim3(kBlock), 0, st, hist_g, cells, P, CH,
                           cell_start, slab_lo, occ_bits, cell_min);
        RPT_TRY(exclusive_scan_total_i32(cell_min, cell_root, cells, st));
        hipLaunchKernelGGL(k_occ_write, dim3(gc), dim3(kBlock), 0, st, cell_min, cell_root,
                           cells, occ);
        hipLaunchKernelGGL(k_cell_start_end, dim3(1), dim3(64), 0, st, cell_start, cells);
        hipLaunchKernelGGL(k_slab_occ_base, dim3(grid_for(nt + 1, kBlock, 1024)), dim3(kBlock), 0,
                           st, cell_root, P, nt, occ_base);
        RPT_CHECK_LAUNCH();
      }
      hipLaunchKernelGGL(k_slab_chunk_scatter, dim3((unsigned)(nt * CH)), dim3(kBucketBlock),
                         hist_bytes, st, x, y, stride, t, g, slab_lo, CH, hist_g, pts, sorig,
                         skey, spos_w);
    } else {
      bucket_allmin = k5_fused_path() && 2 * hist_bytes <= 65536 &&
                      ab_mode("RPT_BUCKET_ALLMIN") != 0;
      const size_t lds = bucket_allmin ? 2 * hist_bytes : hist_bytes;
      RPT_HIP(hipFuncSetAttribute((const void*)k_slab_bucket,
                                  hipFuncAttributeMaxDynamicSharedMemorySize, (int)lds));
#ifdef RPT_AB
      if (ab_env("RPT_STATS")) {
        int nb = -1;
        (void)hipOccupancyMaxActiveBlocksPerMultiprocessor(&nb, k_slab_bucket, kBucketBlock, lds);
        std::fprintf(stderr, "[rpt stats] slab_bucket lds=%zu nx=%d ny=%d blocks_per_cu=%d\n", lds,
                     (int)nx, (int)ny, nb);
      }
#endif
      hipLaunchKernelGGL(k_slab_bucket, dim3((unsigned)nt), dim3(kBucketBlock), lds, st, x, y,
                         stride, t, g, slab_lo, pts, sorig, skey, spos_w, cell_start, hpos,
                         slab_occ,
                         occ_bits,
                         bucket_allmin ? reinterpret_cast<unsigned long long*>(cell_min_pair)
                                       : nullptr);
    }
    RPT_CHECK_LAUNCH();
    if (coalesced_scan) {
      n_occ_dev = occ_base + nt;
    } else {
      RPT_TRY(exclusive_scan_total_i32(slab_occ, occ_base, nt, st));
      hipLaunchKernelGGL(k_occ_gather, dim3((unsigned)nt), dim3(kBlock), 0, st, hpos, slab_lo,
                         occ_base, occ);
      RPT_CHECK_LAUNCH();
      n_occ_dev = occ_base + nt;
    }
  } else {
    hipLaunchKernelGGL(k_keys<D>, dim3(gb), dim3(kBlock), 0, st, x, y, z, stride, t, n, g, keys,
                       vals);
    RPT_CHECK_LAUNCH();
    int bits = 1;
    while ((int64_t(1) << bits) <= C1) ++bits;
    uint32_t *sk, *sv;
    RPT_TRY(radix_sort_pairs(keys, vals, keys_alt, vals_alt, n, bits, rtmp, &sk, &sv, st));
    dense_slabs = false;
    spos_on = label_core_orig() == 2;
    hipLaunchKernelGGL(k_gather<D>, dim3(gb), dim3(kBlock), 0, st, x, y, z, stride, t, n, sk, sv,
                       pts, sorig, skey, spos_on ? slab : nullptr);
    RPT_HIP(hipMemsetAsync(cell_start, 0, sizeof(int32_t) * C1, st));
    hipLaunchKernelGGL(k_cell_runs, dim3(gb), dim3(kBlock), 0, st, skey, n, cell_start, hpos);
    RPT_CHECK_LAUNCH();
    RPT_TRY(exclusive_scan_total_i32(cell_start, cell_start, C1, st));
    RPT_TRY(exclusive_scan_total_i32(hpos, hpos, n, st));
    RPT_HIP(hipMemsetAsync(occ_bits, 0, sizeof(uint32_t) * (C1 / 32 + 2), st));
    hipLaunchKernelGGL(k_occ_list, dim3(gb), dim3(kBlock), 0, st, skey, n, hpos, occ, occ_bits);
    RPT_CHECK_LAUNCH();
    n_occ_dev = hpos + n;
  }
  {
    auto* cmin_w = bucket_allmin ? nullptr : reinterpret_cast<unsigned long long*>(cell_min_pair);
    const int32_t* so_w = (k5_fused_path() && !bucket_allmin) ? (const int32_t*)sorig : nullptr;
    if (cell_box_mixed() == 2 ||
        (cell_box_mixed() == 1 && !dense_slabs && n > (int64_t(1) << 24)))
      hipLaunchKernelGGL(k_cell_box_mixed<D>, dim3(grid_for(n, kBlock, 4096)), dim3(kBlock), 0, st,
                         pts, cell_start, occ, n_occ_dev, g, mutual, cr, cmin_w, so_w);
    else
      hipLaunchKernelGGL(k_cell_box<D>, dim3(grid_for(kCbLanes * n, kBlock, 8192)), dim3(kBlock),
                         0, st, pts, cell_start, occ, n_occ_dev, g, mutual, cr, cmin_w, so_w);
  }
  RPT_CHECK_LAUNCH();
  hipLaunchKernelGGL(k_slab_range<D>, dim3((unsigned)nt), dim3(kBlock), 0, st, cr, occ, hpos,
                     cell_start, (int64_t)(C / nt), (int)nt, slab_t, bucket ? occ_base : nullptr);
  RPT_CHECK_LAUNCH();
  tm.mark();
  return RPT_OK;
}

int32_t DbscanState::build(const float* x, const float* y, const float* z, int64_t stride,
                           const float* t, int64_t n_, double eps_space, double eps_time,
                           int32_t ms, bool timing, hipStream_t st) {
  n = n_;
  dim = z ? 3 : 2;
  min_samples = ms;
  tm.start(timing, st);
  degenerate = !(eps_space >= 0.0) || !((float)eps_time >= 0.0f);
  if (degenerate) return RPT_OK;
  return dim == 2 ? build_t<2>(x, y, z, stride, t, eps_space, eps_time, st)
                  : build_t<3>(x, y, z, stride, t, eps_space, eps_time, st);
}

int32_t DbscanState::core_pass(hipStream_t st) {
  cmin_ready = false;
  if (degenerate) return RPT_OK;
  int32_t* cflag = rep;
  int32_t* cq = ccmin;
  int32_t* n_cq = cid + n;
  int32_t* slow = nc_list;
  int32_t* n_slow = nc_list + n;
  const int32_t* n_occ = n_occ_dev;
  k5_env();
  const double rs = slab_reach();
  const bool oct = oct_ok();
#ifdef RPT_AB
  if (oct && k5_tiles) {
    const int R = (int)rs, W = 2 * R + 1;
    const int by = std::min({8, kTileMap / (W * g.nx) - 4, kTileUnd / g.nx});
    const int64_t nrows = (int64_t)g.nt * g.ny;
    if (by >= 1) {
      hipLaunchKernelGGL(k_row_occ, dim3(grid_for(nrows, kBlock, 4096)), dim3(kBlock), 0, st,
                         occ_bits, nrows, g.nx, rowcnt);
      RPT_CHECK_LAUNCH();
      RPT_TRY(exclusive_scan_total_i32(rowcnt, rowq, nrows, st));
      rowq_ok = true;
      const int nbands = (g.ny + by - 1) / by;
      tile_by = by;
      tile_nbands = nbands;
      tile_R = R;
      const int64_t ntiles = (int64_t)g.nt * nbands;
      const unsigned grid = (unsigned)(((ntiles + 1) + 7) & ~(int64_t)7);
      hipLaunchKernelGGL(k_core_tiles, dim3(grid), dim3(kTileBlock), 0, st, g, R, by, nbands,
                         ntiles, occ, n_occ, rowq, rec<2>(), mutual, occ_bits, slab_t, pts, core);
      RPT_CHECK_LAUNCH();
      tm.mark();
      return RPT_OK;
    }
  }
  if (!k5_legacy) {
    if (oct) {
      hipLaunchKernelGGL(k_core_cells_oct<false>, dim3((grid_for(8 * n, kBlock, 8192) + 7) & ~7), dim3(kBlock), 0,
                         st, g, (int)rs, occ, n_occ, rec<2>(), mutual, occ_bits, slab_t, cflag,
                         (int32_t*)nullptr, k5_fill ? (uint8_t*)nullptr : core);
      if (k5_fill)
        hipLaunchKernelGGL(k_core_fill<false>, dim3(tile_grid(n)), dim3(kBlock), 0, st, skey, n,
                           cflag, core, slow, n_slow);
    } else {
      RPT_TRY(zero_n(st, 1, &n_cq));
      hipLaunchKernelGGL(k_core_cell_fast, dim3(tile_grid(n)), dim3(kBlock), 0, st, occ, n_occ,
                         g, cell_start, mutual, cflag, cq, n_cq);
      if (dim == 2)
        hipLaunchKernelGGL(k_core_cell_window<2>, dim3(wave_grid(n)), dim3(kBlock), 0, st, g,
                           occ, rec<2>(), occ_bits, slab_t, cq, n_cq, cflag);
      else
        hipLaunchKernelGGL(k_core_cell_window<3>, dim3(wave_grid(n)), dim3(kBlock), 0, st, g,
                           occ, rec<3>(), occ_bits, slab_t, cq, n_cq, cflag);
      hipLaunchKernelGGL(k_core_fill<false>, dim3(tile_grid(n)), dim3(kBlock), 0, st, skey, n,
                         cflag, core, slow, n_slow);
    }
    const int gs = wave_grid(n);
    if (dim == 2)
      hipLaunchKernelGGL(k_core_slow_cells<2>, dim3(gs), dim3(kBlock), 0, st, pts, g, rec<2>(),
                         occ_bits, slab_t, occ, n_occ, cflag, core);
    else
      hipLaunchKernelGGL(k_core_slow_cells<3>, dim3(gs), dim3(kBlock), 0, st, pts, g, rec<3>(),
                         occ_bits, slab_t, occ, n_occ, cflag, core);
    RPT_CHECK_LAUNCH();
    tm.mark();
    return RPT_OK;
  }
#endif
  auto* cm = oct ? reinterpret_cast<unsigned long long*>(cell_min_pair) : nullptr;
  if (k5_fused_path()) {
    RPT_TRY(zero_n(st, 1, &n_slow));
    const bool masked = (int)rs <= 2 && k5_mask();
    uint4* k5m = reinterpret_cast<uint4*>(pmask);
    if (masked) {
      hipLaunchKernelGGL((k_core_cells_oct<true, true>),
                         dim3((grid_for(8 * n, kBlock, 8192) + 7) & ~7), dim3(kBlock), 0, st, g,
                         (int)rs, occ, n_occ, rec<2>(), mutual, occ_bits, slab_t,
                         (int32_t*)nullptr, (int32_t*)nullptr, core, cm, slow, cq, n_slow, k5m,
                         cid);
      hipLaunchKernelGGL(k_core_slow_masked, dim3(wave_grid(n)), dim3(kBlock), 0, st, pts, g,
                         (int)rs, rec<2>(), occ, slow, cq, n_slow, k5m, cid, core, sorig, cm);
    } else {
      hipLaunchKernelGGL(k_core_cells_oct<true>, dim3((grid_for(8 * n, kBlock, 8192) + 7) & ~7),
                         dim3(kBlock), 0, st, g, (int)rs, occ, n_occ, rec<2>(), mutual, occ_bits,
                         slab_t, (int32_t*)nullptr, (int32_t*)nullptr, core, cm, slow, cq,
                         n_slow);
    }
    if (masked) {
    } else if (g.rt >= 0 && (2 * g.rt + 1) * 25 <= 128)
      hipLaunchKernelGGL((k_core_slow<2, 2>), dim3(wave_grid(n)), dim3(kBlock), 0, st, pts, skey,
                         g, rec<2>(), occ_bits, slab_t, slow, n_slow, core, sorig, cm, cq);
    else
      hipLaunchKernelGGL(k_core_slow<2>, dim3(wave_grid(n)), dim3(kBlock), 0, st, pts, skey, g,
                         rec<2>(), occ_bits, slab_t, slow, n_slow, core, sorig, cm, cq);
    RPT_CHECK_LAUNCH();
    cmin_ready = true;
#ifdef RPT_AB
    if (ab_env("RPT_STATS")) {
      int32_t h = 0;
      (void)hipMemcpyAsync(&h, n_slow, 4, hipMemcpyDeviceToHost, st);
      (void)hipStreamSynchronize(st);
      std::vector<int32_t> keys((size_t)std::max(h, 0));
      if (h > 0) (void)hipMemcpy(keys.data(), cq, sizeof(int32_t) * (size_t)h, hipMemcpyDeviceToHost);
      std::sort(keys.begin(), keys.end());
      int64_t distinct = 0, max_run = 0, run = 0;
      for (size_t i = 0; i < keys.size(); ++i) {
        run = (i > 0 && keys[i] == keys[i - 1]) ? run + 1 : 1;
        if (run == 1) ++distinct;
        max_run = std::max(max_run, run);
      }
      std::fprintf(stderr, "[rpt stats] n=%lld k5_slow_queue=%d cells=%lld max_per_cell=%lld\n",
                   (long long)n, h, (long long)distinct, (long long)max_run);
    }
#endif
    tm.mark();
    return RPT_OK;
  }
  if (oct) {
    hipLaunchKernelGGL(k_core_cells_oct<false>, dim3((grid_for(8 * n, kBlock, 8192) + 7) & ~7), dim3(kBlock), 0,
                       st, g, (int)rs, occ, n_occ, rec<2>(), mutual, occ_bits, slab_t, cflag,
                       n_slow, (uint8_t*)nullptr);
  } else {
    RPT_TRY(zero_n(st, 1, &n_slow));
    RPT_TRY(zero_n(st, 1, &n_cq));
    hipLaunchKernelGGL(k_core_cell_fast, dim3(tile_grid(n)), dim3(kBlock), 0, st, occ, n_occ, g,
                       cell_start, mutual, cflag, cq, n_cq);
    if (dim == 2)
      hipLaunchKernelGGL(k_core_cell_window<2>, dim3(wave_grid(n)), dim3(kBlock), 0, st, g, occ,
                         rec<2>(), occ_bits, slab_t, cq, n_cq, cflag);
    else
      hipLaunchKernelGGL(k_core_cell_window<3>, dim3(wave_grid(n)), dim3(kBlock), 0, st, g, occ,
                         rec<3>(), occ_bits, slab_t, cq, n_cq, cflag);
  }
  hipLaunchKernelGGL(k_core_fill<true>, dim3(tile_grid(n)), dim3(kBlock), 0, st, skey, n, cflag,
                     core, slow, n_slow, sorig, cm, C);
  if (dim == 2)
    hipLaunchKernelGGL(k_core_slow<2>, dim3(wave_grid(n)), dim3(kBlock), 0, st, pts, skey, g,
                       rec<2>(), occ_bits, slab_t, slow, n_slow, core, sorig, cm);
  else
    hipLaunchKernelGGL(k_core_slow<3>, dim3(wave_grid(n)), dim3(kBlock), 0, st, pts, skey, g,
                       rec<3>(), occ_bits, slab_t, slow, n_slow, core);
  RPT_CHECK_LAUNCH();
  cmin_ready = cm != nullptr;
  tm.mark();
  return RPT_OK;
}

int32_t DbscanState::union_pass(hipStream_t st, bool fused) {
  cell_comp = false;
  if (degenerate) return RPT_OK;
  if (uf_flags < 0) {
    const char* e = ab_env("RPT_UF_FLAGS");
    uf_flags = e ? (std::atoi(e) & 3) : kDefaultUfFlags;
  }
  const int gb = grid_for(n, kBlock, 2048);
  const int gc = grid_for(C, kBlock, 8192);
  const int gw = wave_grid(n);
  const unsigned gp = (unsigned)((n + kBlock - 1) / kBlock);
  const int32_t* n_occ = n_occ_dev;
  (void)gc;
  auto* cmin = reinterpret_cast<unsigned long long*>(cell_min_pair);
  if (union_list < 0) {
    const char* e = ab_env("RPT_UNION_LIST");
    union_list = (e && std::atoi(e) == 0) ? 0 : 1;
  }
  if (union_pair < 0) {
    const char* e = ab_env("RPT_UNION_PAIR");
    union_pair = (e && std::atoi(e) == 0) ? 0 : 1;
  }
  const bool listing = union_list && dim == 2;
  int32_t* plist = listing ? nc_list : nullptr;
  int32_t* pcount = listing ? nc_list + n : nullptr;
  if (union_nm < 0) {
    const char* e = ab_env("RPT_UNION_NM");
    union_nm = (e && std::atoi(e) == 0) ? 0 : 1;
  }
  const bool nm = dim == 2 && union_pair && union_nm;
  int32_t* nm_list = nm ? cid : nullptr;
  int32_t* nm_count = nm ? cid + n : nullptr;
  if (uf_compress < 0) {
    const char* e = ab_env("RPT_UF_COMPRESS");
    uf_compress = (e && std::atoi(e) == 1) ? 1 : 0;
  }
  cell_comp = fused && all_mutual && listing && nm && cell_comp_enabled() && !use_label_tiles() &&
              !uf_compress;
  if (!cell_comp || !cmin_ready)
    hipLaunchKernelGGL(k_init_occ_cells, dim3(gb), dim3(kBlock), 0, st, occ, n_occ, C, rep,
                       cmin_ready ? nullptr : cmin, pcount, nm_count);
  if (!cmin_ready)
    hipLaunchKernelGGL(k_cell_min_pair, dim3(gb), dim3(kBlock), 0, st, skey, core, sorig, n, C,
                       cmin);
  if (cell_comp)
    hipLaunchKernelGGL(k_parent_init_cells, dim3(gb), dim3(kBlock), 0, st, occ, n_occ, C, cmin,
                       rep, parent, pcount, nm_count, min_bits, min_words(), cell_min);
  else
    hipLaunchKernelGGL(k_parent_init_pair, dim3(grid_for(n, kBlock * kPU, 2048)), dim3(kBlock), 0,
                       st, parent, n, core, skey, mutual, cmin, C, rep);
  int32_t* lstat_dev = nullptr;
  if (dim == 2) {
    uint4* pm = listing ? pmask : nullptr;
    if (union_pair)
      hipLaunchKernelGGL(k_union_cells_pair, dim3(gw), dim3(kBlock), 0, st, pts, g, occ, n_occ,
                         rec<2>(), occ_bits, slab_t, rep, mutual, sorig, parent, uf_flags, pm,
                         plist, pcount, union_cpw(), nm_list, nm_count);
    else
      hipLaunchKernelGGL((k_union_cells<2, false>), dim3(gw), dim3(kBlock), 0, st, pts, g,
                         cell_start, occ, n_occ, rec<2>(), occ_bits, slab_t, core, rep, mutual,
                         sorig, parent, uf_flags, pm, plist, pcount);
#ifdef RPT_AB
    if (listing && ab_env("RPT_STATS")) {
      static int32_t* buf = nullptr;
      if (!buf) (void)hipMalloc(&buf, 16);
      lstat_dev = buf;
      (void)hipMemsetAsync(lstat_dev, 0, 16, st);
    }
#endif
    if (listing) {
      const bool snap = union_snapshot() == 2 || (union_snapshot() == 1 && !dense_slabs);
      if (snap)
        hipLaunchKernelGGL(k_cell_root_snapshot, dim3(grid_for(n, kBlock, 4096)), dim3(kBlock),
                           0, st, occ, n_occ, rep, parent, g.cells, uf_flags, cell_root);
      hipLaunchKernelGGL(k_union_listed, dim3(gw), dim3(kBlock), 0, st, pts, g, occ, rec<2>(),
                         occ_bits, slab_t, core, rep, mutual, sorig, parent, uf_flags, pm, plist,
                         pcount, snap ? (const int32_t*)cell_root : nullptr, lstat_dev);
    }
    else
      hipLaunchKernelGGL((k_union_cells<2, true>), dim3(gw), dim3(kBlock), 0, st, pts, g,
                         cell_start, occ, n_occ, rec<2>(), occ_bits, slab_t, core, rep, mutual,
                         sorig, parent, uf_flags, pm, plist, pcount);
    if (cell_comp) {
    } else if (nm)
      hipLaunchKernelGGL(k_union_nm<2>, dim3(gw), dim3(kBlock), 0, st, pts, g, cell_start,
                         rec<2>(), slab_t, core, rep, mutual, sorig, parent, nm_list, nm_count);
    else
      hipLaunchKernelGGL(k_union<2>, dim3(gp), dim3(kBlock), 0, st, pts, skey, n, g, cell_start,
                         rec<2>(), slab_t, core, rep, mutual, sorig, parent);
  } else {
    hipLaunchKernelGGL((k_union_cells<3, false>), dim3(gw), dim3(kBlock), 0, st, pts, g,
                       cell_start, occ, n_occ, rec<3>(), occ_bits, slab_t, core, rep, mutual, sorig,
                       parent, uf_flags);
    hipLaunchKernelGGL((k_union_cells<3, true>), dim3(gw), dim3(kBlock), 0, st, pts, g,
                       cell_start, occ, n_occ, rec<3>(), occ_bits, slab_t, core, rep, mutual, sorig,
                       parent, uf_flags);
    hipLaunchKernelGGL(k_union<3>, dim3(gp), dim3(kBlock), 0, st, pts, skey, n, g, cell_start,
                       rec<3>(), slab_t, core, rep, mutual, sorig, parent);
  }
  RPT_CHECK_LAUNCH();
#ifdef RPT_AB
  if (uf_compress && !cell_comp)
    hipLaunchKernelGGL(k_compress, dim3(gb), dim3(kBlock), 0, st, parent, core, n, sorig,
                       (int32_t*)nullptr);
  if (ab_env("RPT_STATS")) {
    int32_t h[2] = {0, 0}, ls[4] = {0, 0, 0, 0};
    (void)hipMemcpyAsync(&h[0], n_occ_dev, 4, hipMemcpyDeviceToHost, st);
    if (listing) (void)hipMemcpyAsync(&h[1], pcount, 4, hipMemcpyDeviceToHost, st);
    if (lstat_dev) (void)hipMemcpyAsync(ls, lstat_dev, 16, hipMemcpyDeviceToHost, st);
    (void)hipStreamSynchronize(st);
    std::fprintf(stderr,
                 "[rpt stats] n=%lld occupied=%d listed_cells=%d listed: undecided=%d "
                 "roots_differ=%d searches=%d hits=%d\n",
                 (long long)n, h[0], h[1], ls[0], ls[1], ls[2], ls[3]);
    std::fprintf(stderr, "[rpt stats] n=%lld all_mutual=%d cell_comp=%d\n", (long long)n,
                 all_mutual ? 1 : 0, cell_comp ? 1 : 0);
  }
#endif
  RPT_CHECK_LAUNCH();
  tm.mark();
  return RPT_OK;
}

int32_t DbscanState::cluster_ids(hipStream_t st, int32_t* cell_key, int32_t* zero) {
  const int64_t W = min_words();
  const bool cr = cell_roots_enabled();
  if (cr) {
    hipLaunchKernelGGL(k_cell_roots, dim3(grid_for(n, kBlock, 2048)), dim3(kBlock), 0, st, parent,
                       occ, n_occ_dev, C, mutual, rep, cell_root, zero, min_bits, W, cell_key);
  } else {
    RPT_HIP(hipMemsetAsync(min_bits, 0, sizeof(uint32_t) * W, st));
    if (zero) RPT_HIP(hipMemsetAsync(zero, 0, sizeof(int32_t), st));
    if (cell_key)
      hipLaunchKernelGGL(k_fill_i32, dim3(grid_for(C, kBlock, 8192)), dim3(kBlock), 0, st,
                         cell_key, C, INT_MAX);
  }
  hipLaunchKernelGGL(k_ccmin, dim3(tile_grid(n)), dim3(kBlock), 0, st, parent, core, n, sorig,
                     ccmin, min_bits, nc_list, nc_list + n, skey, mutual,
                     cr ? (const int32_t*)cell_root : nullptr, C, cell_key);
  hipLaunchKernelGGL(k_word_popc, dim3(grid_for(W, kBlock, 2048)), dim3(kBlock), 0, st, min_bits,
                     W, min_pref);
  RPT_CHECK_LAUNCH();
  return exclusive_scan_total_i32(min_pref, min_pref, W, st);
}

int32_t DbscanState::labels_local(int32_t* labels, rpt_stdbscan_stats* stats, hipStream_t st) {
  const int gb = grid_for(n, kBlock, 2048);
  if (degenerate) {
    hipLaunchKernelGGL(k_isolated_labels, dim3(gb), dim3(kBlock), 0, st, labels, n,
                       min_samples <= 0 ? 1 : 0);
    RPT_CHECK_LAUNCH();
    if (stats) {
      stats->n_points = n;
      stats->n_core = min_samples <= 0 ? n : 0;
      stats->n_clusters = min_samples <= 0 ? (int32_t)n : 0;
    }
    return RPT_OK;
  }
  int32_t* nc_count = nc_list + n;
  const MinRank mr{min_bits, min_pref};
  const unsigned glc = (unsigned)((grid_for(n, kBlock * kPU, 2048) + 7) & ~7);
  if (cell_comp) {
    const int64_t W = min_words();
    hipLaunchKernelGGL(k_cell_comp, dim3(grid_for(n, kBlock, 2048)), dim3(kBlock), 0, st, parent,
                       occ, n_occ_dev, C, rep, sorig, cell_min, min_bits, nc_count);
    hipLaunchKernelGGL(k_word_popc, dim3(grid_for(W, kBlock, 2048)), dim3(kBlock), 0, st,
                       min_bits, W, min_pref);
    RPT_CHECK_LAUNCH();
    RPT_TRY(exclusive_scan_total_i32(min_pref, min_pref, W, st));
    if (spos_on)
      hipLaunchKernelGGL(k_label_core_cells<true>, dim3(glc), dim3(kBlock), 0, st, skey, core,
                         slab, n, C, cell_min, mr, labels, nc_list, nc_count, cid + n,
                         n_clusters_ptr());
    else
      hipLaunchKernelGGL(k_label_core_cells<false>, dim3(glc), dim3(kBlock), 0, st, skey, core,
                         sorig, n, C, cell_min, mr, labels, nc_list, nc_count, cid + n,
                         n_clusters_ptr());
  } else {
    RPT_TRY(cluster_ids(st, cell_min, nc_count));
    if (spos_on)
      hipLaunchKernelGGL(k_label_core_orig, dim3(glc), dim3(kBlock), 0, st, ccmin, n, slab, mr,
                         labels);
    else
      hipLaunchKernelGGL(k_label_core, dim3(glc), dim3(kBlock), 0, st, ccmin, n, sorig, mr,
                         labels);
  }
  int32_t* kstat = nullptr;
#ifdef RPT_AB
  if (ab_env("RPT_STATS")) {
    static int32_t* buf = nullptr;
    if (!buf) (void)hipMalloc(&buf, 16);
    kstat = buf;
    (void)hipMemsetAsync(kstat, 0, 16, st);
  }
#endif
#ifdef RPT_AB
  if (use_label_tiles())
    hipLaunchKernelGGL((k_label_tiles<false>), dim3(tile_grid_blocks()), dim3(kTileBlock), 0, st,
                       g, tile_R, tile_by, tile_nbands, (int64_t)g.nt * tile_nbands, occ,
                       n_occ_dev, rowq, rec<2>(), mutual, occ_bits, slab_t, pts, ccmin, cell_min,
                       sorig, mr, min_samples, labels);
  else if (cell_comp && label_w() == 64)
    hipLaunchKernelGGL((k_label<2, false, 64, true>), dim3(wave_grid(n)), dim3(kBlock), 0, st,
                       pts, skey, g, rec<2>(), occ_bits, slab_t, (const int32_t*)nullptr,
                       cell_min, mutual, sorig, mr, nc_list, nc_count, labels,
                       (int32_t*)nullptr, core);
  else if (dim == 2 && label_w() == 64)
    hipLaunchKernelGGL((k_label<2, false, 64>), dim3(wave_grid(n)), dim3(kBlock), 0, st, pts,
                       skey, g, rec<2>(), occ_bits, slab_t, ccmin, cell_min, mutual, sorig, mr,
                       nc_list, nc_count, labels);
  else
#endif
  if (cell_comp)
    hipLaunchKernelGGL((k_label<2, false, 32, true>), dim3(wave_grid(n)), dim3(kBlock), 0, st,
                       pts, skey, g, rec<2>(), occ_bits, slab_t, (const int32_t*)nullptr,
                       cell_min, mutual, sorig, mr, nc_list, nc_count, labels, kstat, core);
  else if (dim == 2)
    hipLaunchKernelGGL((k_label<2, false, 32>),
                       dim3(wave_grid(n)), dim3(kBlock), 0, st, pts, skey, g,
                       rec<2>(), occ_bits, slab_t, ccmin, cell_min, mutual, sorig, mr, nc_list,
                       nc_count, labels, kstat);
  else
    hipLaunchKernelGGL((k_label<3, false, 64>),
                       dim3(wave_grid(n)), dim3(kBlock), 0, st, pts, skey, g,
                       rec<3>(), occ_bits, slab_t, ccmin, cell_min, mutual, sorig, mr, nc_list,
                       nc_count, labels);
  RPT_CHECK_LAUNCH();
#ifdef RPT_AB
  if (kstat) {
    int32_t ks[4] = {0, 0, 0, 0};
    (void)hipMemcpyAsync(ks, kstat, 16, hipMemcpyDeviceToHost, st);
    (void)hipStreamSynchronize(st);
    std::fprintf(stderr,
                 "[rpt stats] n=%lld label: queued=%d core_in_window=%d searched=%d labelled=%d\n",
                 (long long)n, ks[0], ks[1], ks[2], ks[3]);
  }
#endif
  tm.mark();
  if (stats && defer) return RPT_OK;
  if (stats) {
    int32_t ncl = 0;
    RPT_HIP(hipMemcpyAsync(&ncl, n_clusters_ptr(), sizeof(int32_t), hipMemcpyDeviceToHost, st));
    RPT_TRY(wait_stream(st));
    RPT_TRY(fill_stats(ncl, stats));
  }
  return RPT_OK;
}

int32_t DbscanState::fill_stats(int32_t ncl, rpt_stdbscan_stats* stats) {
  if (ncl < 0) {
    set_error("rpt_stdbscan: a non-mutual cell on a grid taken for all-mutual (labels invalid)");
    return RPT_EHIP;
  }
  {
    stats->n_points = n;
    stats->n_clusters = ncl;
    stats->n_core = -1;
    stats->grid_dims[0] = g.nx;
    stats->grid_dims[1] = g.ny;
    stats->grid_dims[2] = g.nz;
    stats->grid_dims[3] = g.nt;
    stats->grid_cells = C;
    if (tm.on && tm.k >= 6) {
      RPT_HIP(hipEventSynchronize(tm.ev[tm.k - 1]));
      stats->ms_bounds = tm.ms(0);
      stats->ms_grid = tm.ms(1);
      stats->ms_core = tm.ms(2);
      stats->ms_union = tm.ms(3);
      stats->ms_label = tm.ms(4);
    }
  }
  return RPT_OK;
}

int32_t DbscanState::labels_global(const int64_t* rep_orig, const int64_t* reps, int64_t nr,
                                   int32_t* labels, hipStream_t st, const int64_t* nr_dev) {
  if (degenerate) {
    set_error("rpt_dbscan_labels_global: degenerate parameters are handled by rpt_stdbscan");
    return RPT_ENOTSUP;
  }
  const int gb = grid_for(n, kBlock, 2048);
  int32_t* nc_count = nc_list + n;
  const bool cr = cell_roots_enabled();
  if (cr) {
    hipLaunchKernelGGL(k_cell_roots, dim3(grid_for(n, kBlock, 2048)), dim3(kBlock), 0, st, parent,
                       occ, n_occ_dev, C, mutual, rep, cell_root, nc_count, (uint32_t*)nullptr,
                       (int64_t)0, cell_min);
  } else {
    RPT_HIP(hipMemsetAsync(nc_count, 0, sizeof(int32_t), st));
    hipLaunchKernelGGL(k_fill_i32, dim3(grid_for(C, kBlock, 8192)), dim3(kBlock), 0, st, cell_min,
                       C, INT_MAX);
  }
  hipLaunchKernelGGL(k_ccmin_global, dim3(tile_grid(n)), dim3(kBlock), 0, st, parent, core, n,
                     sorig, rep_orig, reps, nr, ccmin, cid, nc_list, nc_count, skey, mutual,
                     cr ? (const int32_t*)cell_root : nullptr, C, nr_dev);
  const bool orig = spos_on;
  if (orig)
    hipLaunchKernelGGL(k_label_global_orig, dim3(grid_for(n, kBlock * kPU, 2048)), dim3(kBlock), 0,
                       st, core, ccmin, cid, slab, n, labels);
  hipLaunchKernelGGL(k_label_global_core, dim3(gb), dim3(kBlock), 0, st, core, ccmin, cid, sorig,
                     n, slab, orig ? nullptr : labels, skey, C, cell_min);
  spos_on = false;
#ifdef RPT_AB
  if (use_label_tiles())
    hipLaunchKernelGGL((k_label_tiles<true>), dim3(tile_grid_blocks()), dim3(kTileBlock), 0, st,
                       g, tile_R, tile_by, tile_nbands, (int64_t)g.nt * tile_nbands, occ,
                       n_occ_dev, rowq, rec<2>(), mutual, occ_bits, slab_t, pts, slab, cell_min,
                       sorig, MinRank{nullptr, nullptr}, min_samples, labels);
  else if (dim == 2 && label_w() == 64)
    hipLaunchKernelGGL((k_label<2, true, 64>), dim3(wave_grid(n)), dim3(kBlock), 0, st, pts,
                       skey, g, rec<2>(), occ_bits, slab_t, slab, cell_min, mutual, sorig,
                       MinRank{nullptr, nullptr}, nc_list, nc_count, labels);
  else
#endif
  if (dim == 2)
    hipLaunchKernelGGL((k_label<2, true, 32>),
                       dim3(wave_grid(n)), dim3(kBlock), 0, st, pts, skey, g,
                       rec<2>(), occ_bits, slab_t, slab, cell_min, mutual, sorig,
                       MinRank{nullptr, nullptr}, nc_list, nc_count, labels);
  else
    hipLaunchKernelGGL((k_label<3, true, 64>),
                       dim3(wave_grid(n)), dim3(kBlock), 0, st, pts, skey, g,
                       rec<3>(), occ_bits, slab_t, slab, cell_min, mutual, sorig,
                       MinRank{nullptr, nullptr}, nc_list, nc_count, labels);
  RPT_CHECK_LAUNCH();
  return RPT_OK;
}

int32_t DbscanState::frames_pass(int32_t min_frames, hipStream_t st) {
  if (degenerate || min_frames < 1) return RPT_OK;
  cmin_ready = false;
  const bool refine = min_frames >= 2;
  int32_t* list = nc_list;
  int32_t* count = nc_list + n;
  const int32_t* n_occ = n_occ_dev;
  const bool cells = refine && integral_t && dim == 2 && g.nz == 1;
  const int one_frame_cells = (integral_t && g.ct == 1.0) ? 1 : 0;
  if (cells) {
    const int R = (int)std::min<double>(std::floor((double)g.epst / g.ct), 64.0);
    hipLaunchKernelGGL(k_frames_cells, dim3(grid_for(n, kBlock, 8192)), dim3(kBlock), 0, st, g, R,
                       occ, n_occ, rec<2>(), occ_bits, min_frames, fok);
  }
  RPT_TRY(zero_n(st, 1, &count));
  hipLaunchKernelGGL(k_frames_queue, dim3(tile_grid(n)), dim3(kBlock), 0, st, skey, n, C,
                     cells ? (const uint8_t*)fok : (const uint8_t*)nullptr, (int)min_frames,
                     refine ? 1 : 0, core, list, count);
  if (refine) {
    const bool small = (double)g.epst <= 30.0;
    if (dim == 2 && small)
      hipLaunchKernelGGL(k_frames_points<2>, dim3(wave_grid(n)), dim3(kBlock), 0, st, pts, skey, g,
                         rec<2>(), occ_bits, slab_t, one_frame_cells, (int)min_frames, list,
                         count, core);
    else if (small)
      hipLaunchKernelGGL(k_frames_points<3>, dim3(wave_grid(n)), dim3(kBlock), 0, st, pts, skey, g,
                         rec<3>(), occ_bits, slab_t, one_frame_cells, (int)min_frames, list,
                         count, core);
    else if (dim == 2)
      hipLaunchKernelGGL(k_frames_points_list<2>, dim3(wave_grid(n)), dim3(kBlock), 0, st, pts,
                         skey, g, rec<2>(), occ_bits, slab_t, one_frame_cells,
                         (int)min_frames, list, count, core);
    else
      hipLaunchKernelGGL(k_frames_points_list<3>, dim3(wave_grid(n)), dim3(kBlock), 0, st, pts,
                         skey, g, rec<3>(), occ_bits, slab_t, one_frame_cells,
                         (int)min_frames, list, count, core);
  }
  RPT_CHECK_LAUNCH();
  return RPT_OK;
}

int32_t DbscanState::labels_fifo(int32_t* labels, rpt_stdbscan_stats* stats, hipStream_t st) {
  int32_t* nc_count = nc_list + n;
  int32_t* spos = slab;
  RPT_TRY(cluster_ids(st, nullptr, nc_count));
  if (!spos_on)
    hipLaunchKernelGGL(k_inverse_perm, dim3(grid_for(n, kBlock, 2048)), dim3(kBlock), 0, st,
                       sorig, n, spos);
  const MinRank mr{min_bits, min_pref};
  hipLaunchKernelGGL(k_label_core_orig, dim3((grid_for(n, kBlock * kPU, 2048) + 7) & ~7),
                     dim3(kBlock), 0, st, ccmin, n, spos, mr, labels);
  if (dim == 2)
    hipLaunchKernelGGL((k_label_fifo<2>), dim3(wave_grid(n)), dim3(kBlock), 0, st, pts, skey, g,
                       rec<2>(), occ_bits, slab_t, ccmin, rep, sorig, spos, mr, nc_list,
                       nc_count, labels);
  else
    hipLaunchKernelGGL((k_label_fifo<3>), dim3(wave_grid(n)), dim3(kBlock), 0, st, pts, skey, g,
                       rec<3>(), occ_bits, slab_t, ccmin, rep, sorig, spos, mr, nc_list,
                       nc_count, labels);
  RPT_CHECK_LAUNCH();
  tm.mark();
  int32_t ncl = 0;
  RPT_HIP(hipMemcpyAsync(&ncl, n_clusters_ptr(), sizeof(int32_t), hipMemcpyDeviceToHost, st));
  RPT_TRY(wait_stream(st));
  if (stats) RPT_TRY(fill_stats(ncl, stats));
  return RPT_OK;
}

static int32_t check_args(const float* x, const float* y, const float* z, int64_t stride,
                          const float* t, int64_t n, int dim) {
  if (n <= 0) {
    set_error("Found array with 0 sample(s) (shape=(0, %d)) while a minimum of 1 is required.",
              dim);
    return RPT_EEMPTY;
  }
  if (n >= (int64_t(1) << 31) - 2) {
    set_error("rpt_stdbscan: n=%lld exceeds the int32 index space", (long long)n);
    return RPT_ENOTSUP;
  }
  if (!x || !y || !t || (dim == 3 && !z) || stride < 1) {
    set_error("rpt_stdbscan: null pointer or bad stride");
    return RPT_EINVAL;
  }
  return RPT_OK;
}

static std::mutex g_state_mu;
static std::vector<std::pair<std::pair<int, hipStream_t>, DbscanState*>> g_states;

int32_t stdbscan(const float* x, const float* y, const float* z, int64_t stride, const float* t,
                 int64_t n, double eps_space, double eps_time, int32_t min_samples,
                 int32_t* labels, rpt_stdbscan_stats* stats, hipStream_t st, int dim) {
  RPT_TRY(check_args(x, y, z, stride, t, n, dim));
  if (!labels) {
    set_error("rpt_stdbscan: null labels");
    return RPT_EINVAL;
  }
  int dev = 0;
  RPT_HIP(hipGetDevice(&dev));
  DbscanState* S;
  {
    std::lock_guard<std::mutex> lk(g_state_mu);
    S = nullptr;
    for (auto& e : g_states)
      if (e.first.first == dev && e.first.second == st) S = e.second;
    if (!S) {
      S = new DbscanState();
      g_states.push_back({{dev, st}, S});
    }
  }
  RPT_TRY(S->build(x, y, z, stride, t, n, eps_space, eps_time, min_samples,
                   stats && stats->timing, st));
  RPT_TRY(S->core_pass(st));
  RPT_TRY(S->union_pass(st, stats != nullptr));
  return S->labels_local(labels, stats, st);
}

int32_t stdbscan_denoise(const float* x, const float* y, const float* t, int64_t n,
                         double eps_space, double eps_time, int32_t min_samples,
                         int32_t min_frames, int32_t* labels, rpt_stdbscan_stats* stats,
                         hipStream_t st) {
  if (n == 0) {
    if (stats) *stats = rpt_stdbscan_stats{};
    return RPT_OK;
  }
  RPT_TRY(check_args(x, y, nullptr, 1, t, n, 2));
  if (!labels) {
    set_error("rpt_stdbscan_denoise: null labels");
    return RPT_EINVAL;
  }
  if (min_frames > 64 * kFramesPerLane && !((float)eps_time <= 30.0f) &&
      (float)eps_time == (float)eps_time) {
    set_error("rpt_stdbscan_denoise: min_frames > %d with eps_time > 30 is not supported",
              64 * kFramesPerLane);
    return RPT_ENOTSUP;
  }
  int dev = 0;
  RPT_HIP(hipGetDevice(&dev));
  DbscanState* S;
  {
    std::lock_guard<std::mutex> lk(g_state_mu);
    S = nullptr;
    for (auto& e : g_states)
      if (e.first.first == dev && e.first.second == st) S = e.second;
    if (!S) {
      S = new DbscanState();
      g_states.push_back({{dev, st}, S});
    }
  }
  RPT_TRY(S->build(x, y, nullptr, 1, t, n, eps_space, eps_time, min_samples,
                   stats && stats->timing, st));
  if (S->degenerate) {
    const bool single = min_samples <= 0 && min_frames <= 0;
    hipLaunchKernelGGL(k_isolated_labels, dim3(grid_for(n, kBlock, 2048)), dim3(kBlock), 0, st,
                       labels, n, single ? 1 : 0);
    RPT_CHECK_LAUNCH();
    if (stats) {
      stats->n_points = n;
      stats->n_core = single ? n : 0;
      stats->n_clusters = single ? (int32_t)n : 0;
    }
    return wait_stream(st);
  }
  RPT_TRY(S->core_pass(st));
  RPT_TRY(S->frames_pass(min_frames, st));
  RPT_TRY(S->union_pass(st));
  return S->labels_fifo(labels, stats, st);
}

size_t stdbscan_bounds_bytes() { return sizeof(Bounds); }
int32_t stdbscan_bounds_dev(const float* x, const float* y, const float* t, int64_t n_max,
                            const int64_t* n_dev, void* out_dev, void* part_dev,
                            hipStream_t st) {
  const int nbb = grid_for(std::max<int64_t>(n_max, 1), kBlock, 1024);
  hipLaunchKernelGGL(k_bounds<2>, dim3(nbb), dim3(kBlock), 0, st, x, y, (const float*)nullptr,
                     (int64_t)1, t, n_max, static_cast<Bounds*>(part_dev), n_dev);
  hipLaunchKernelGGL(k_bounds_final, dim3(1), dim3(kBlock), 0, st,
                     static_cast<const Bounds*>(part_dev), nbb, static_cast<Bounds*>(out_dev));
  RPT_CHECK_LAUNCH();
  return RPT_OK;
}
int32_t stdbscan_bounds_final_dev(const void* part_dev, int nb, void* out_dev, hipStream_t st) {
  hipLaunchKernelGGL(k_bounds_final, dim3(1), dim3(kBlock), 0, st,
                     static_cast<const Bounds*>(part_dev), nb, static_cast<Bounds*>(out_dev));
  RPT_CHECK_LAUNCH();
  return RPT_OK;
}
static_assert(kBlock == kBoundsBlock, "k_bounds is launched with kBlock threads per block");
size_t stdbscan_bounds_part_bytes(int64_t n_max) {
  return sizeof(Bounds) * (size_t)grid_for(std::max<int64_t>(n_max, 1), kBoundsBlock, 1024);
}

int32_t stdbscan_deferred(const float* x, const float* y, const float* z, int64_t stride,
                          const float* t, int64_t n, double eps_space, double eps_time,
                          int32_t min_samples, int32_t* labels, rpt_stdbscan_stats* stats,
                          hipStream_t st, int dim, const int32_t** n_clusters_dev,
                          void** state, const void* host_bounds) {
  RPT_TRY(check_args(x, y, z, stride, t, n, dim));
  if (!labels || !stats || !n_clusters_dev || !state) {
    set_error("stdbscan_deferred: null argument");
    return RPT_EINVAL;
  }
  int dev = 0;
  RPT_HIP(hipGetDevice(&dev));
  DbscanState* S;
  {
    std::lock_guard<std::mutex> lk(g_state_mu);
    S = nullptr;
    for (auto& e : g_states)
      if (e.first.first == dev && e.first.second == st) S = e.second;
    if (!S) {
      S = new DbscanState();
      g_states.push_back({{dev, st}, S});
    }
  }
  S->given_bounds = host_bounds;
  const int32_t sb = S->build(x, y, z, stride, t, n, eps_space, eps_time, min_samples,
                              stats->timing != 0, st);
  S->given_bounds = nullptr;
  RPT_TRY(sb);
  RPT_TRY(S->core_pass(st));
  RPT_TRY(S->union_pass(st, true));
  S->defer = !S->degenerate;
  const int32_t s_ = S->labels_local(labels, stats, st);
  *n_clusters_dev = S->defer ? S->n_clusters_ptr() : nullptr;
  *state = S;
  return s_;
}

int32_t stdbscan_core_flags(void* state, int64_t n, uint8_t* out, hipStream_t st) {
  DbscanState* S = static_cast<DbscanState*>(state);
  if (!S || S->degenerate || S->n != n || !S->core || !S->sorig) {
    set_error("rpt_stack_core_flags: no core flags for this run");
    return RPT_EINVAL;
  }
  hipLaunchKernelGGL(k_core_to_orig, dim3(grid_for(n, kBlock, 2048)), dim3(kBlock), 0, st,
                     S->core, S->sorig, n, out);
  RPT_CHECK_LAUNCH();
  return RPT_OK;
}

int32_t stdbscan_fill_stats(void* state, int32_t n_clusters, rpt_stdbscan_stats* stats) {
  DbscanState* S = static_cast<DbscanState*>(state);
  S->defer = false;
  return S->fill_stats(n_clusters, stats);
}

DbscanState* dbscan_create() { return new DbscanState(); }
void dbscan_destroy(DbscanState* s) {
  if (s) {
    s->arena.release();
    delete s;
  }
}
int32_t dbscan_build(DbscanState* S, const float* x, const float* y, const float* z,
                     int64_t stride, const float* t, int64_t n, double eps_space,
                     double eps_time, int32_t ms, hipStream_t st) {
  RPT_TRY(check_args(x, y, z, stride, t, n, z ? 3 : 2));
  RPT_TRY(S->build(x, y, z, stride, t, n, eps_space, eps_time, ms, false, st));
  if (S->degenerate) {
    set_error("rpt_dbscan_build: negative or NaN eps (use rpt_stdbscan)");
    return RPT_ENOTSUP;
  }
  return RPT_OK;
}
int32_t dbscan_core(DbscanState* S, uint8_t* core_out, hipStream_t st) {
  RPT_TRY(S->core_pass(st));
  if (core_out) {
    hipLaunchKernelGGL(k_core_to_orig, dim3(grid_for(S->n, kBlock, 2048)), dim3(kBlock), 0, st,
                       S->core, S->sorig, S->n, core_out);
    RPT_CHECK_LAUNCH();
  }
  return RPT_OK;
}
int32_t dbscan_set_core(DbscanState* S, const uint8_t* core_in, hipStream_t st) {
  S->cmin_ready = false;
  hipLaunchKernelGGL(k_core_from_orig, dim3(grid_for(S->n, kBlock, 2048)), dim3(kBlock), 0, st,
                     core_in, S->sorig, S->n, S->core);
  RPT_CHECK_LAUNCH();
  return RPT_OK;
}
int32_t dbscan_components(DbscanState* S, int32_t* comp_out, hipStream_t st) {
  RPT_TRY(S->union_pass(st));
  if (S->degenerate || S->n == 0) {
    hipLaunchKernelGGL(k_comp_out, dim3(grid_for(S->n, kBlock, 2048)), dim3(kBlock), 0, st,
                       S->parent, S->core, S->sorig, S->n, comp_out, S->skey,
                       (const int32_t*)nullptr, (int64_t)0);
  } else {
    hipLaunchKernelGGL(k_cell_roots, dim3(grid_for(S->n, kBlock, 2048)), dim3(kBlock), 0, st,
                       S->parent, S->occ, S->n_occ_dev, S->C, S->mutual, S->rep, S->cell_root,
                       (int32_t*)nullptr);
    hipLaunchKernelGGL(k_comp_out, dim3(grid_for(S->n, kBlock, 2048)), dim3(kBlock), 0, st,
                       S->parent, S->core, S->sorig, S->n, comp_out, S->skey,
                       (const int32_t*)S->cell_root, S->C);
  }
  RPT_CHECK_LAUNCH();
  return RPT_OK;
}
int32_t dbscan_components_edges(DbscanState* S, int32_t* comp_out, int64_t lo_end,
// ... 95 lines not shown
```

Before: 7678.

## Store 2-D points as float2 when each time slab holds a single timestamp

Adds an xy-only point layout (float2 instead of float4) used when every slab holds a single time value, so per-cell time bounds come from a per-slab time table and the time checks in adjacency and classification are skipped. This is meant to halve point-buffer traffic in bucketing, cell-box, core, union and label kernels, and to drop the z/t reductions and the slab-range kernel. It adds template variants and guards (need_float4) that fall back or fail on paths that still need the time component, which adds risk that a path silently depends on the float4 layout.

```diff
diff --git a/radar-point-cloud-tracking_amd/csrc/stdbscan.hip b/radar-point-cloud-tracking_amd/csrc/stdbscan.hip
--- a/radar-point-cloud-tracking_amd/csrc/stdbscan.hip
+++ b/radar-point-cloud-tracking_amd/csrc/stdbscan.hip
@@ -279,6 +279,39 @@
   return cell_of((double)t, g.ot, g.inv_ct, g.nt);
 }
 
+template <bool XY>
+struct PtRec {
+  using type = float4;
+};
+template <>
+struct PtRec<true> {
+  using type = float2;
+};
+template <bool XY>
+using Pt = typename PtRec<XY>::type;
+template <bool XY>
+__device__ __forceinline__ float4 load_pt(const Pt<XY>* __restrict__ pts, int64_t i) {
+  if constexpr (XY) {
+    const float2 v = pts[i];
+    return make_float4(v.x, v.y, NAN, NAN);
+  } else {
+    return pts[i];
+  }
+}
+template <bool XY>
+__device__ __forceinline__ void store_pt(Pt<XY>* __restrict__ pts, int64_t i, float x, float y,
+                                         float t) {
+  if constexpr (XY)
+    pts[i] = make_float2(x, y);
+  else
+    pts[i] = make_float4(x, y, t, t);
+}
+__device__ __forceinline__ float2 slab_time_of(const float* __restrict__ t, int lo, int hi) {
+  if (lo >= hi) return make_float2(FLT_MAX, -FLT_MAX);
+  const float v = t[lo];
+  return make_float2(v, v);
+}
+
 template <int D>
 __global__ __launch_bounds__(kBlock) void k_keys(const float* __restrict__ x,
                                                 const float* __restrict__ y,
@@ -447,19 +480,21 @@
   }
 }
 
+template <bool XY>
 __global__ __launch_bounds__(kBucketBlock) void k_slab_bucket(
     const float* __restrict__ x, const float* __restrict__ y, int64_t stride,
     const float* __restrict__ t, Geom g, const int32_t* __restrict__ slab_lo,
-    float4* __restrict__ pts, int32_t* __restrict__ sorig, int32_t* __restrict__ skey,
+    Pt<XY>* __restrict__ pts, int32_t* __restrict__ sorig, int32_t* __restrict__ skey,
     int32_t* __restrict__ spos, int32_t* __restrict__ cell_start, int32_t* __restrict__ occ_tmp,
     int32_t* __restrict__ slab_occ, uint32_t* __restrict__ occ_bits,
-    unsigned long long* __restrict__ cmin_all = nullptr) {
+    unsigned long long* __restrict__ cmin_all, float2* __restrict__ slab_t) {
   extern __shared__ int32_t hist[];
   __shared__ int32_t wsum[kBucketBlock / 64], wocc[kBucketBlock / 64];
   const int s = blockIdx.x;
   const int P = g.nx * g.ny;
   int32_t* mn = hist + P;
   const int lo = slab_lo[s], hi = slab_lo[s + 1];
+  if (XY && threadIdx.x == 0) slab_t[s] = slab_time_of(t, lo, hi);
   for (int c = threadIdx.x; c < P; c += kBucketBlock) {
     hist[c] = 0;
     if (cmin_all) mn[c] = INT_MAX;
@@ -564,7 +599,7 @@
       const int i = min(i0 + u * kBucketBlock + (int)threadIdx.x, hi - 1);
       px[u] = x[(int64_t)i * stride];
       py[u] = y[(int64_t)i * stride];
-      pt[u] = t[i];
+      pt[u] = XY ? 0.f : t[i];
     }
 #pragma unroll
     for (int u = 0; u < kBucketU; ++u) {
@@ -577,7 +612,7 @@
       base = __shfl(base, head, 64);
       if (v) {
         const int dst = lo + base + rank;
-        pts[dst] = make_float4(px[u], py[u], pt[u], pt[u]);
+        store_pt<XY>(pts, dst, px[u], py[u], pt[u]);
         sorig[dst] = i;
         if (spos) spos[i] = dst;
         skey[dst] = s * P + c;
@@ -752,17 +787,19 @@
     if (occf[k]) occ[pos[k]] = (int32_t)k;
 }
 
+template <bool XY>
 __global__ __launch_bounds__(kBucketBlock) void k_slab_chunk_scatter(
     const float* __restrict__ x, const float* __restrict__ y, int64_t stride,
     const float* __restrict__ t, Geom g, const int32_t* __restrict__ slab_lo, int CH,
-    const int32_t* __restrict__ hist_g, float4* __restrict__ pts, int32_t* __restrict__ sorig,
-    int32_t* __restrict__ skey, int32_t* __restrict__ spos) {
+    const int32_t* __restrict__ hist_g, Pt<XY>* __restrict__ pts, int32_t* __restrict__ sorig,
+    int32_t* __restrict__ skey, int32_t* __restrict__ spos, float2* __restrict__ slab_t) {
   extern __shared__ int32_t cur[];
   const int s = blockIdx.x / CH, ch = blockIdx.x - s * CH;
   const int P = g.nx * g.ny;
   int lo, hi;
   slab_chunk(slab_lo, s, ch, CH, lo, hi);
   const int base = slab_lo[s];
+  if (XY && ch == 0 && threadIdx.x == 0) slab_t[s] = slab_time_of(t, base, slab_lo[s + 1]);
   const int32_t* hc = hist_g + (int64_t)blockIdx.x * P;
   for (int c = threadIdx.x; c < P; c += kBucketBlock) cur[c] = hc[c];
   __syncthreads();
@@ -773,7 +810,7 @@
       const int i = min(i0 + u * kBucketBlock + (int)threadIdx.x, hi - 1);
       px[u] = x[(int64_t)i * stride];
       py[u] = y[(int64_t)i * stride];
-      pt[u] = t[i];
+      pt[u] = XY ? 0.f : t[i];
     }
 #pragma unroll
     for (int u = 0; u < kBucketU; ++u) {
@@ -782,7 +819,7 @@
         const int c = cell_of((double)py[u], g.oy, g.inv_cs, g.ny) * g.nx +
                       cell_of((double)px[u], g.ox, g.inv_cs, g.nx);
         const int dst = base + atomicAdd(&cur[c], 1);
-        pts[dst] = make_float4(px[u], py[u], pt[u], pt[u]);
+        store_pt<XY>(pts, dst, px[u], py[u], pt[u]);
         sorig[dst] = i;
         if (spos) spos[i] = dst;
         skey[dst] = s * P + c;
@@ -879,8 +916,8 @@
 }
 
 constexpr int kCbLanes = 16;
-template <int D>
-__global__ __launch_bounds__(kBlock) void k_cell_box(const float4* __restrict__ pts,
+template <int D, bool XY = false>
+__global__ __launch_bounds__(kBlock) void k_cell_box(const Pt<XY>* __restrict__ pts,
                                                     const int32_t* __restrict__ cell_start,
                                                     const int32_t* __restrict__ occ,
                                                     const int32_t* __restrict__ n_occ, Geom g,
@@ -888,7 +925,9 @@
                                                     CellRec<D>* __restrict__ crec,
                                                     unsigned long long* __restrict__ cmin =
                                                         nullptr,
-                                                    const int32_t* __restrict__ sorig = nullptr) {
+                                                    const int32_t* __restrict__ sorig = nullptr,
+                                                    const float2* __restrict__ slab_t = nullptr) {
+  static_assert(!XY || D == 2, "xy points are 2-D");
   constexpr int L = kCbLanes;
   const int j = threadIdx.x & (L - 1);
   const int64_t no = *n_occ;
@@ -913,7 +952,7 @@
       for (int u = 0; u < kU; ++u) {
         const int s2 = s0 + L * u;
         const int sc = (s2 < e) ? s2 : s0;
-        pp[u] = pts[sc];
+        pp[u] = load_pt<XY>(pts, sc);
         if (sorig) so[u] = (uint32_t)sorig[sc];
       }
 #pragma unroll
@@ -921,8 +960,10 @@
         const float4 p = pp[u];
         x0 = fminf(x0, p.x); x1 = fmaxf(x1, p.x);
         y0 = fminf(y0, p.y); y1 = fmaxf(y1, p.y);
-        z0 = fminf(z0, p.z); z1 = fmaxf(z1, p.z);
-        t0 = fminf(t0, p.w); t1 = fmaxf(t1, p.w);
+        if constexpr (!XY) {
+          z0 = fminf(z0, p.z); z1 = fmaxf(z1, p.z);
+          t0 = fminf(t0, p.w); t1 = fmaxf(t1, p.w);
+        }
         if (sorig) {
           const int s2 = s0 + L * u;
           const uint64_t v = ((uint64_t)so[u] << 32) | (uint32_t)((s2 < e) ? s2 : s0);
@@ -933,8 +974,12 @@
     if (sorig) mn = row_reduce<L>(mn, OpMin{});
     x0 = row_reduce<L>(x0, OpMin{}); x1 = row_reduce<L>(x1, OpMax{});
     y0 = row_reduce<L>(y0, OpMin{}); y1 = row_reduce<L>(y1, OpMax{});
-    z0 = row_reduce<L>(z0, OpMin{}); z1 = row_reduce<L>(z1, OpMax{});
-    t0 = row_reduce<L>(t0, OpMin{}); t1 = row_reduce<L>(t1, OpMax{});
+    if constexpr (XY) {
+      t0 = t1 = slab_t[g.slab_of_key(c)].x;
+    } else {
+      z0 = row_reduce<L>(z0, OpMin{}); z1 = row_reduce<L>(z1, OpMax{});
+      t0 = row_reduce<L>(t0, OpMin{}); t1 = row_reduce<L>(t1, OpMax{});
+    }
     if (D != 3) {
       z0 = t0;
       z1 = t1;
@@ -1002,8 +1047,8 @@
   if (cmin) cmin[c] = has_mn ? mn : ~0ull;
 }
 
-template <int D>
-__global__ __launch_bounds__(kBlock) void k_cell_box_mixed(const float4* __restrict__ pts,
+template <int D, bool XY = false>
+__global__ __launch_bounds__(kBlock) void k_cell_box_mixed(const Pt<XY>* __restrict__ pts,
                                                           const int32_t* __restrict__ cell_start,
                                                           const int32_t* __restrict__ occ,
                                                           const int32_t* __restrict__ n_occ,
@@ -1012,7 +1057,10 @@
                                                           unsigned long long* __restrict__ cmin =
                                                               nullptr,
                                                           const int32_t* __restrict__ sorig =
+                                                              nullptr,
+                                                          const float2* __restrict__ slab_t =
                                                               nullptr) {
+  static_assert(!XY || D == 2, "xy points are 2-D");
   constexpr int L = kCbLanes;
   const int lane = threadIdx.x & 63;
   const int grp = lane / L, j = lane & (L - 1);
@@ -1032,19 +1080,22 @@
 #pragma unroll
       for (int u = 0; u < kCbSmall; ++u) {
         const int sc = (b + u < e) ? b + u : b;
-        pp[u] = pts[sc];
+        pp[u] = load_pt<XY>(pts, sc);
         if (sorig) so[u] = (uint32_t)sorig[sc];
       }
       float x0 = FLT_MAX, x1 = -FLT_MAX, y0 = FLT_MAX, y1 = -FLT_MAX;
       float z0 = FLT_MAX, z1 = -FLT_MAX, t0 = FLT_MAX, t1 = -FLT_MAX;
+      if constexpr (XY) t0 = t1 = slab_t[g.slab_of_key(c)].x;
       uint64_t mn = ~0ull;
 #pragma unroll
       for (int u = 0; u < kCbSmall; ++u) {
         const float4 p = pp[u];
         x0 = fminf(x0, p.x); x1 = fmaxf(x1, p.x);
         y0 = fminf(y0, p.y); y1 = fmaxf(y1, p.y);
-        z0 = fminf(z0, p.z); z1 = fmaxf(z1, p.z);
-        t0 = fminf(t0, p.w); t1 = fmaxf(t1, p.w);
+        if constexpr (!XY) {
+          z0 = fminf(z0, p.z); z1 = fmaxf(z1, p.z);
+          t0 = fminf(t0, p.w); t1 = fmaxf(t1, p.w);
+        }
         if (sorig) {
           const uint64_t v = ((uint64_t)so[u] << 32) | (uint32_t)((b + u < e) ? b + u : b);
           mn = v < mn ? v : mn;
@@ -1081,7 +1132,7 @@
         for (int u = 0; u < kU; ++u) {
           const int s2 = s0 + L * u;
           const int sc = (s2 < ee) ? s2 : s0;
-          pp[u] = pts[sc];
+          pp[u] = load_pt<XY>(pts, sc);
           if (sorig) so[u] = (uint32_t)sorig[sc];
         }
 #pragma unroll
@@ -1089,8 +1140,10 @@
           const float4 p = pp[u];
           x0 = fminf(x0, p.x); x1 = fmaxf(x1, p.x);
           y0 = fminf(y0, p.y); y1 = fmaxf(y1, p.y);
-          z0 = fminf(z0, p.z); z1 = fmaxf(z1, p.z);
-          t0 = fminf(t0, p.w); t1 = fmaxf(t1, p.w);
+          if constexpr (!XY) {
+            z0 = fminf(z0, p.z); z1 = fmaxf(z1, p.z);
+            t0 = fminf(t0, p.w); t1 = fmaxf(t1, p.w);
+          }
           if (sorig) {
             const int s2 = s0 + L * u;
             const uint64_t v = ((uint64_t)so[u] << 32) | (uint32_t)((s2 < ee) ? s2 : s0);
@@ -1101,8 +1154,12 @@
       if (sorig) mn = row_reduce<L>(mn, OpMin{});
       x0 = row_reduce<L>(x0, OpMin{}); x1 = row_reduce<L>(x1, OpMax{});
       y0 = row_reduce<L>(y0, OpMin{}); y1 = row_reduce<L>(y1, OpMax{});
-      z0 = row_reduce<L>(z0, OpMin{}); z1 = row_reduce<L>(z1, OpMax{});
-      t0 = row_reduce<L>(t0, OpMin{}); t1 = row_reduce<L>(t1, OpMax{});
+      if constexpr (XY) {
+        t0 = t1 = slab_t[g.slab_of_key(cc)].x;
+      } else {
+        z0 = row_reduce<L>(z0, OpMin{}); z1 = row_reduce<L>(z1, OpMax{});
+        t0 = row_reduce<L>(t0, OpMin{}); t1 = row_reduce<L>(t1, OpMax{});
+      }
       if (D != 3) {
         z0 = t0;
         z1 = t1;
@@ -1153,9 +1210,9 @@
 }
 
 
-template <int D>
+template <int D, bool XY = false>
 __device__ __forceinline__ bool adjacent(const float4& a, const float4& b, const Geom& g) {
-  const float dt = fabsf(a.w - b.w);
+  const float dt = XY ? 0.f : fabsf(a.w - b.w);
   const float fx = a.x - b.x, fy = a.y - b.y;
   float f2 = fx * fx + fy * fy;
   if (D == 3) {
@@ -1174,7 +1231,7 @@
     }
     in = d2 <= g.eps2;
   }
-  return in && (dt <= g.epst);
+  return XY ? in : (in && (dt <= g.epst));
 }
 
 __device__ __forceinline__ void span_dist(float p, float lo, float hi, double& dmin,
@@ -1184,13 +1241,16 @@
   dmax = fmax(fabs(dp - (double)lo), fabs(dp - (double)hi));
 }
 
-template <int D>
+template <int D, bool XY = false>
 __device__ __forceinline__ int classify(const float4& p, const float4& A, const float4& B,
                                         const Geom& g) {
-  const float tlo = B.z, thi = B.w;
-  const float tmin = (p.w < tlo) ? (tlo - p.w) : ((p.w > thi) ? (p.w - thi) : 0.f);
-  if (!(tmin <= g.epst)) return 0;
-  const float tmax = fmaxf(fabsf(p.w - tlo), fabsf(p.w - thi));
+  float tmax = 0.f;
+  if constexpr (!XY) {
+    const float tlo = B.z, thi = B.w;
+    const float tmin = (p.w < tlo) ? (tlo - p.w) : ((p.w > thi) ? (p.w - thi) : 0.f);
+    if (!(tmin <= g.epst)) return 0;
+    tmax = fmaxf(fabsf(p.w - tlo), fabsf(p.w - thi));
+  }
   {
     auto fgap = [](float v, float lo, float hi) { return fmaxf(fmaxf(lo - v, v - hi), 0.f); };
     auto fspan = [](float v, float lo, float hi) { return fmaxf(fabsf(v - lo), fabsf(v - hi)); };
@@ -1384,6 +1444,18 @@
 }
 
 template <int D>
+__device__ __forceinline__ Window slab_window(int cx, int cy, int cz, int s, const Geom& g) {
+  Window w;
+  w.s0 = max(s - g.rt, 0);
+  w.nS = max(min(s + g.rt, g.nt - 1) - w.s0 + 1, 0);
+  w.x0 = cx - 2;
+  w.y0 = cy - 2;
+  w.z0 = (D == 3) ? cz - 2 : 0;
+  w.total = w.nS * ((D == 3) ? 125 : 25);
+  return w;
+}
+
+template <int D>
 __device__ __forceinline__ void decode_key(int64_t key, const Geom& g, int& cx, int& cy, int& cz) {
   int cs;
   g.split((uint32_t)key, cx, cy, cz, cs);
@@ -1409,7 +1481,9 @@
   return (((int64_t)sl * g.nz + z) * g.ny + y) * g.nx + x;
 }
 
+template <bool XY = false>
 __device__ __forceinline__ float4 shfl_f4(const float4& v, int l) {
+  if constexpr (XY) return make_float4(__shfl(v.x, l), __shfl(v.y, l), NAN, NAN);
   return make_float4(__shfl(v.x, l), __shfl(v.y, l), __shfl(v.z, l), __shfl(v.w, l));
 }
 
@@ -2018,8 +2092,9 @@
   const int y = cy + cw_row(k) - 2;
   return (s2 * g.ny + y) * g.nx + (cx - 2 + dx);
 }
+template <bool XY>
 __global__ __launch_bounds__(kBlock, 8) void k_core_slow_masked(
-    const float4* __restrict__ pts, Geom g, int R, const CellRec<2>* __restrict__ crec,
+    const Pt<XY>* __restrict__ pts, Geom g, int R, const CellRec<2>* __restrict__ crec,
     const int32_t* __restrict__ occ, const int32_t* __restrict__ slow,
     const int32_t* __restrict__ slowq, const int32_t* __restrict__ n_slow,
     const uint4* __restrict__ pmask, const int32_t* __restrict__ clo, uint8_t* __restrict__ core,
@@ -2032,7 +2107,7 @@
   for (int64_t q = xr.first; q < xr.end; q += xr.step) {
     const int s = slow[q];
     const int32_t cq = slowq[q];
-    const float4 p = pts[s];
+    const float4 p = load_pt<XY>(pts, s);
     const int32_t key = occ[cq];
     const uint4 m = pmask[cq];
     int cnt = clo[cq];
@@ -2044,8 +2119,8 @@
     const int k0 = h0 ? mask_pos_key(lane, g, R, W, mg, cx, cy, cs) : key;
     const int k1 = h1 ? mask_pos_key(lane + 64, g, R, W, mg, cx, cy, cs) : key;
     const CellRec<2> c0 = crec[k0], c1 = crec[k1];
-    const int cl0 = h0 ? classify<2>(p, rec_boxA<2>(c0), rec_boxB(c0), g) : 0;
-    const int cl1 = h1 ? classify<2>(p, rec_boxA<2>(c1), rec_boxB(c1), g) : 0;
+    const int cl0 = h0 ? classify<2, XY>(p, rec_boxA<2>(c0), rec_boxB(c0), g) : 0;
+    const int cl1 = h1 ? classify<2, XY>(p, rec_boxA<2>(c1), rec_boxB(c1), g) : 0;
     int add = (cl0 == 1 ? c0.e - c0.b : 0) + (cl1 == 1 ? c1.e - c1.b : 0);
     int may = (cl0 == 2 ? c0.e - c0.b : 0) + (cl1 == 2 ? c1.e - c1.b : 0);
     cnt += wave_sum(add);
@@ -2061,7 +2136,7 @@
           const int bb = __shfl(bq, l), ee = __shfl(eq, l);
           for (int j0 = bb; j0 < ee && cnt < need; j0 += 64) {
             const int jj = j0 + lane;
-            const bool a = (jj < ee) && adjacent<2>(p, pts[jj], g);
+            const bool a = (jj < ee) && adjacent<2, XY>(p, load_pt<XY>(pts, jj), g);
             cnt += __popcll(__ballot(a));
           }
         }
@@ -2595,7 +2670,8 @@
   }
 }
 
-__global__ __launch_bounds__(kBlock) void k_union_listed(const float4* __restrict__ pts, Geom g,
+template <bool XY>
+__global__ __launch_bounds__(kBlock) void k_union_listed(const Pt<XY>* __restrict__ pts, Geom g,
                                                         const int32_t* __restrict__ occ,
                                                         const CellRec<2>* __restrict__ crec,
                                                         const uint32_t* __restrict__ occ_bits,
@@ -2660,21 +2736,21 @@
           float4 pb = make_float4(0.f, 0.f, 0.f, 0.f);
           bool cb_ok = false;
           if (jb < ebl && core[jb]) {
-            pb = pts[jb];
-            cb_ok = classify<2>(pb, A1, A2, g) != 0;
+            pb = load_pt<XY>(pts, jb);
+            cb_ok = classify<2, XY>(pb, A1, A2, g) != 0;
           }
           const uint64_t bm = __ballot(cb_ok);
           for (int ja0 = ba; bm && ja0 < ea && !hit; ja0 += 64) {
             const int ja = ja0 + lane;
             const bool va = (ja < ea) && core[ja];
-            const float4 pa = va ? pts[ja] : make_float4(0.f, 0.f, 0.f, 0.f);
+            const float4 pa = va ? load_pt<XY>(pts, ja) : make_float4(0.f, 0.f, 0.f, 0.f);
             bool adj = false;
             uint64_t rest = bm;
             while (rest) {
               const int lb = __ffsll((unsigned long long)rest) - 1;
               rest &= rest - 1;
-              const float4 pq = shfl_f4(pb, lb);
-              adj = adj || (va && adjacent<2>(pq, pa, g));
+              const float4 pq = shfl_f4<XY>(pb, lb);
+              adj = adj || (va && adjacent<2, XY>(pq, pa, g));
             }
             hit = __ballot(adj) != 0;
           }
@@ -3123,8 +3199,8 @@
   }
 }
 
-template <int D, bool GLOBAL, int W = 64, bool ALLMUT = false>
-__global__ __launch_bounds__(kBlock, 6) void k_label(const float4* __restrict__ pts,
+template <int D, bool GLOBAL, int W = 64, bool ALLMUT = false, bool XY = false>
+__global__ __launch_bounds__(kBlock, 6) void k_label(const Pt<XY>* __restrict__ pts,
                                                  const int32_t* __restrict__ skey, Geom g,
                                                  const CellRec<D>* __restrict__ crec,
                                                  const uint32_t* __restrict__ occ_bits,
@@ -3140,6 +3216,7 @@
                                                  int32_t* __restrict__ kstat = nullptr,
                                                  const uint8_t* __restrict__ core_of = nullptr) {
   static_assert(!ALLMUT || (D == 2 && !GLOBAL), "all-mutual grids are 2-D, local runs");
+  static_assert(!XY || ALLMUT, "xy points only on all-mutual grids");
   static_assert(W == 32 || W == 64, "a point per wave or per half-wave");
   constexpr int P = 64 / W;
   const int lane = threadIdx.x & 63;
@@ -3168,10 +3245,11 @@
     bool st_core = false, st_search = false;
 #endif
     if ((int64_t)key < g.cells) {
-      const float4 p = pts[s];
+      const float4 p = load_pt<XY>(pts, s);
       int cx, cy, cz;
       decode_key<D>(key, g, cx, cy, cz);
-      const Window w = make_window<D, false>(cx, cy, cz, p.w, p.w, g, slab_t);
+      const Window w = XY ? slab_window<D>(cx, cy, cz, g.slab_of_key(key), g)
+                          : make_window<D, false>(cx, cy, cz, p.w, p.w, g, slab_t);
       for (int base = 0; base < w.total; base += W * kR) {
         int64_t c[kR];
         int ck[kR], cb[kR], ce[kR], cls[kR], mu[kR];
@@ -3191,7 +3269,7 @@
             cb[k] = cr.b;
             ce[k] = cr.e;
             mu[k] = ALLMUT ? 1 : mutual[c[k]];
-            cls[k] = classify<D>(p, rec_boxA<D>(cr), rec_boxB(cr), g);
+            cls[k] = classify<D, XY>(p, rec_boxA<D>(cr), rec_boxB(cr), g);
             if (cls[k] == 1) v = min(v, ck[k]);
           }
         }
@@ -3246,9 +3324,10 @@
                 k1 = v1 ? key_of[j] : -1;
                 k2 = v2 ? key_of[j2] : -1;
               }
-              const float4 p1 = v1 ? pts[j] : p, p2 = v2 ? pts[j2] : p;
-              hit = gbal((k1 >= 0 && adjacent<D>(p, p1, g)) ||
-                         (k2 >= 0 && adjacent<D>(p, p2, g))) != 0;
+              const float4 p1 = v1 ? load_pt<XY>(pts, j) : p;
+              const float4 p2 = v2 ? load_pt<XY>(pts, j2) : p;
+              hit = gbal((k1 >= 0 && adjacent<D, XY>(p, p1, g)) ||
+                         (k2 >= 0 && adjacent<D, XY>(p, p2, g))) != 0;
             }
             if (hit) best = mm;
           } else {
@@ -3257,9 +3336,10 @@
               const int j = j0 + hl, j2 = j + W;
               const bool v1 = j < el, v2 = j2 < el;
               const int m1 = v1 ? key_of[j] : -1, m2 = v2 ? key_of[j2] : -1;
-              const float4 p1 = v1 ? pts[j] : p, p2 = v2 ? pts[j2] : p;
-              if (m1 >= 0 && m1 < best && m1 < lb && adjacent<D>(p, p1, g)) lb = m1;
-              if (m2 >= 0 && m2 < best && m2 < lb && adjacent<D>(p, p2, g)) lb = m2;
+              const float4 p1 = v1 ? load_pt<XY>(pts, j) : p;
+              const float4 p2 = v2 ? load_pt<XY>(pts, j2) : p;
+              if (m1 >= 0 && m1 < best && m1 < lb && adjacent<D, XY>(p, p1, g)) lb = m1;
+              if (m2 >= 0 && m2 < best && m2 < lb && adjacent<D, XY>(p, p2, g)) lb = m2;
             }
             best = min(best, gmin(lb));
           }
@@ -3888,6 +3968,45 @@
   bool integral_t = false;
   bool all_mutual = false;
   bool cell_comp = false;
+  void union_env() {
+    if (union_list < 0) {
+      const char* e = ab_env("RPT_UNION_LIST");
+      union_list = (e && std::atoi(e) == 0) ? 0 : 1;
+    }
+    if (union_pair < 0) {
+      const char* e = ab_env("RPT_UNION_PAIR");
+      union_pair = (e && std::atoi(e) == 0) ? 0 : 1;
+    }
+    if (union_nm < 0) {
+      const char* e = ab_env("RPT_UNION_NM");
+      union_nm = (e && std::atoi(e) == 0) ? 0 : 1;
+    }
+    if (uf_compress < 0) {
+      const char* e = ab_env("RPT_UF_COMPRESS");
+      uf_compress = (e && std::atoi(e) == 1) ? 1 : 0;
+    }
+  }
+  bool cell_comp_ok() {
+    union_env();
+    return all_mutual && dim == 2 && union_list && union_pair && union_nm &&
+           cell_comp_enabled() && !use_label_tiles() && !uf_compress;
+  }
+  bool xy_points = false;
+  bool may_xy = false;
+  bool xy_rule() {
+    static const bool on = [] {
+      const char* e = ab_env("RPT_XY_POINTS");
+      return !(e && std::atoi(e) == 0);
+    }();
+    (void)use_label_tiles();
+    return on && dim == 2 && g.tfree && g.epst == std::floor(g.epst) && cell_comp_ok() &&
+           k5_fused_path() && (int)slab_reach() <= 2 && k5_mask() && !k7_tiles && label_w() == 32;
+  }
+  int32_t need_float4(const char* who) const {
+    if (!xy_points) return RPT_OK;
+    set_error("%s: internal: this state's sorted points are xy-only", who);
+    return RPT_EHIP;
+  }
   int64_t* stmp = nullptr;
   Timer tm;
 
@@ -4093,6 +4212,8 @@
   bucket_allmin = false;
   const bool bucket = bucket_mode && D == 2 && hb.n_finite_t == n && !hb.t_descends &&
                       (int64_t)nx * ny <= kBucketCells && nt < (int64_t(1) << 31);
+  xy_points = may_xy && bucket && D == 2 && hb.n_finite_t == n && xy_rule();
+  Pt<true>* pts_xy = reinterpret_cast<Pt<true>*>(pts);
   if (bucket) {
     hipLaunchKernelGGL(k_slab_lo, dim3(grid_for(64 * (nt + 1), kBlock, 4096)), dim3(kBlock), 0,
                        st, t, n, g, slab_lo, occ_bits, (int64_t)(C1 / 32 + 2));
@@ -4112,7 +4233,8 @@
       int32_t* hist_g = reinterpret_cast<int32_t*>(keys);
       RPT_HIP(hipFuncSetAttribute((const void*)k_slab_chunk_hist,
                                   hipFuncAttributeMaxDynamicSharedMemorySize, (int)hist_bytes));
-      RPT_HIP(hipFuncSetAttribute((const void*)k_slab_chunk_scatter,
+      RPT_HIP(hipFuncSetAttribute(xy_points ? (const void*)k_slab_chunk_scatter<true>
+                                            : (const void*)k_slab_chunk_scatter<false>,
                                   hipFuncAttributeMaxDynamicSharedMemorySize, (int)hist_bytes));
       hipLaunchKernelGGL(k_slab_chunk_hist, dim3((unsigned)(nt * CH)), dim3(kBucketBlock),
                          hist_bytes, st, x, y, stride, g, slab_lo, CH, hist_g);
@@ -4136,29 +4258,44 @@
                            st, cell_root, P, nt, occ_base);
         RPT_CHECK_LAUNCH();
       }
-      hipLaunchKernelGGL(k_slab_chunk_scatter, dim3((unsigned)(nt * CH)), dim3(kBucketBlock),
-                         hist_bytes, st, x, y, stride, t, g, slab_lo, CH, hist_g, pts, sorig,
-                         skey, spos_w);
+      if (xy_points)
+        hipLaunchKernelGGL(k_slab_chunk_scatter<true>, dim3((unsigned)(nt * CH)),
+                           dim3(kBucketBlock), hist_bytes, st, x, y, stride, t, g, slab_lo, CH,
+                           hist_g, pts_xy, sorig, skey, spos_w, slab_t);
+      else
+        hipLaunchKernelGGL(k_slab_chunk_scatter<false>, dim3((unsigned)(nt * CH)),
+                           dim3(kBucketBlock), hist_bytes, st, x, y, stride, t, g, slab_lo, CH,
+                           hist_g, pts, sorig, skey, spos_w, (float2*)nullptr);
     } else {
       bucket_allmin = k5_fused_path() && 2 * hist_bytes <= 65536 &&
                       ab_mode("RPT_BUCKET_ALLMIN") != 0;
       const size_t lds = bucket_allmin ? 2 * hist_bytes : hist_bytes;
-      RPT_HIP(hipFuncSetAttribute((const void*)k_slab_bucket,
+      RPT_HIP(hipFuncSetAttribute(xy_points ? (const void*)k_slab_bucket<true>
+                                            : (const void*)k_slab_bucket<false>,
                                   hipFuncAttributeMaxDynamicSharedMemorySize, (int)lds));
 #ifdef RPT_AB
       if (ab_env("RPT_STATS")) {
         int nb = -1;
-        (void)hipOccupancyMaxActiveBlocksPerMultiprocessor(&nb, k_slab_bucket, kBucketBlock, lds);
+        if (xy_points)
+          (void)hipOccupancyMaxActiveBlocksPerMultiprocessor(&nb, k_slab_bucket<true>,
+                                                             kBucketBlock, lds);
+        else
+          (void)hipOccupancyMaxActiveBlocksPerMultiprocessor(&nb, k_slab_bucket<false>,
+                                                             kBucketBlock, lds);
         std::fprintf(stderr, "[rpt stats] slab_bucket lds=%zu nx=%d ny=%d blocks_per_cu=%d\n", lds,
                      (int)nx, (int)ny, nb);
       }
 #endif
-      hipLaunchKernelGGL(k_slab_bucket, dim3((unsigned)nt), dim3(kBucketBlock), lds, st, x, y,
-                         stride, t, g, slab_lo, pts, sorig, skey, spos_w, cell_start, hpos,
-                         slab_occ,
-                         occ_bits,
-                         bucket_allmin ? reinterpret_cast<unsigned long long*>(cell_min_pair)
-                                       : nullptr);
+      auto* cmin_all =
+          bucket_allmin ? reinterpret_cast<unsigned long long*>(cell_min_pair) : nullptr;
+      if (xy_points)
+        hipLaunchKernelGGL(k_slab_bucket<true>, dim3((unsigned)nt), dim3(kBucketBlock), lds, st,
+                           x, y, stride, t, g, slab_lo, pts_xy, sorig, skey, spos_w, cell_start,
+                           hpos, slab_occ, occ_bits, cmin_all, slab_t);
+      else
+        hipLaunchKernelGGL(k_slab_bucket<false>, dim3((unsigned)nt), dim3(kBucketBlock), lds, st,
+                           x, y, stride, t, g, slab_lo, pts, sorig, skey, spos_w, cell_start,
+                           hpos, slab_occ, occ_bits, cmin_all, (float2*)nullptr);
     }
     RPT_CHECK_LAUNCH();
     if (coalesced_scan) {
@@ -4195,17 +4332,30 @@
   {
     auto* cmin_w = bucket_allmin ? nullptr : reinterpret_cast<unsigned long long*>(cell_min_pair);
     const int32_t* so_w = (k5_fused_path() && !bucket_allmin) ? (const int32_t*)sorig : nullptr;
-    if (cell_box_mixed() == 2 ||
-        (cell_box_mixed() == 1 && !dense_slabs && n > (int64_t(1) << 24)))
-      hipLaunchKernelGGL(k_cell_box_mixed<D>, dim3(grid_for(n, kBlock, 4096)), dim3(kBlock), 0, st,
-                         pts, cell_start, occ, n_occ_dev, g, mutual, cr, cmin_w, so_w);
+    const bool mixed = cell_box_mixed() == 2 ||
+                       (cell_box_mixed() == 1 && !dense_slabs && n > (int64_t(1) << 24));
+    const dim3 gm(grid_for(n, kBlock, 4096)), gl(grid_for(kCbLanes * n, kBlock, 8192));
+    if (xy_points) {
+      if constexpr (D == 2) {
+        if (mixed)
+          hipLaunchKernelGGL((k_cell_box_mixed<2, true>), gm, dim3(kBlock), 0, st, pts_xy,
+                             cell_start, occ, n_occ_dev, g, mutual, cr, cmin_w, so_w, slab_t);
+        else
+          hipLaunchKernelGGL((k_cell_box<2, true>), gl, dim3(kBlock), 0, st, pts_xy, cell_start,
+                             occ, n_occ_dev, g, mutual, cr, cmin_w, so_w, slab_t);
+      }
+    } else if (mixed)
+      hipLaunchKernelGGL(k_cell_box_mixed<D>, gm, dim3(kBlock), 0, st, pts, cell_start, occ,
+                         n_occ_dev, g, mutual, cr, cmin_w, so_w);
     else
-      hipLaunchKernelGGL(k_cell_box<D>, dim3(grid_for(kCbLanes * n, kBlock, 8192)), dim3(kBlock),
-                         0, st, pts, cell_start, occ, n_occ_dev, g, mutual, cr, cmin_w, so_w);
+      hipLaunchKernelGGL(k_cell_box<D>, gl, dim3(kBlock), 0, st, pts, cell_start, occ, n_occ_dev,
+                         g, mutual, cr, cmin_w, so_w);
   }
   RPT_CHECK_LAUNCH();
-  hipLaunchKernelGGL(k_slab_range<D>, dim3((unsigned)nt), dim3(kBlock), 0, st, cr, occ, hpos,
-                     cell_start, (int64_t)(C / nt), (int)nt, slab_t, bucket ? occ_base : nullptr);
+  if (!xy_points)
+    hipLaunchKernelGGL(k_slab_range<D>, dim3((unsigned)nt), dim3(kBlock), 0, st, cr, occ, hpos,
+                       cell_start, (int64_t)(C / nt), (int)nt, slab_t,
+                       bucket ? occ_base : nullptr);
   RPT_CHECK_LAUNCH();
   tm.mark();
   return RPT_OK;
@@ -4217,6 +4367,11 @@
   n = n_;
   dim = z ? 3 : 2;
   min_samples = ms;
+  xy_points = false;
+  struct Consume {
+    bool& f;
+    ~Consume() { f = false; }
+  } consume{may_xy};
   tm.start(timing, st);
   degenerate = !(eps_space >= 0.0) || !((float)eps_time >= 0.0f);
   if (degenerate) return RPT_OK;
@@ -4236,6 +4391,7 @@
   k5_env();
   const double rs = slab_reach();
   const bool oct = oct_ok();
+  if (!k5_fused_path()) RPT_TRY(need_float4("core_pass"));
 #ifdef RPT_AB
   if (oct && k5_tiles) {
     const int R = (int)rs, W = 2 * R + 1;
@@ -4297,6 +4453,7 @@
   if (k5_fused_path()) {
     RPT_TRY(zero_n(st, 1, &n_slow));
     const bool masked = (int)rs <= 2 && k5_mask();
+    if (!masked) RPT_TRY(need_float4("core_pass"));
     uint4* k5m = reinterpret_cast<uint4*>(pmask);
     if (masked) {
       hipLaunchKernelGGL((k_core_cells_oct<true, true>),
@@ -4304,8 +4461,14 @@
                          (int)rs, occ, n_occ, rec<2>(), mutual, occ_bits, slab_t,
                          (int32_t*)nullptr, (int32_t*)nullptr, core, cm, slow, cq, n_slow, k5m,
                          cid);
-      hipLaunchKernelGGL(k_core_slow_masked, dim3(wave_grid(n)), dim3(kBlock), 0, st, pts, g,
-                         (int)rs, rec<2>(), occ, slow, cq, n_slow, k5m, cid, core, sorig, cm);
+      if (xy_points)
+        hipLaunchKernelGGL(k_core_slow_masked<true>, dim3(wave_grid(n)), dim3(kBlock), 0, st,
+                           reinterpret_cast<const Pt<true>*>(pts), g, (int)rs, rec<2>(), occ,
+                           slow, cq, n_slow, k5m, cid, core, sorig, cm);
+      else
+        hipLaunchKernelGGL(k_core_slow_masked<false>, dim3(wave_grid(n)), dim3(kBlock), 0, st,
+                           pts, g, (int)rs, rec<2>(), occ, slow, cq, n_slow, k5m, cid, core,
+                           sorig, cm);
     } else {
       hipLaunchKernelGGL(k_core_cells_oct<true>, dim3((grid_for(8 * n, kBlock, 8192) + 7) & ~7),
                          dim3(kBlock), 0, st, g, (int)rs, occ, n_occ, rec<2>(), mutual, occ_bits,
@@ -4386,30 +4549,15 @@
   const int32_t* n_occ = n_occ_dev;
   (void)gc;
   auto* cmin = reinterpret_cast<unsigned long long*>(cell_min_pair);
-  if (union_list < 0) {
-    const char* e = ab_env("RPT_UNION_LIST");
-    union_list = (e && std::atoi(e) == 0) ? 0 : 1;
-  }
-  if (union_pair < 0) {
-    const char* e = ab_env("RPT_UNION_PAIR");
-    union_pair = (e && std::atoi(e) == 0) ? 0 : 1;
-  }
+  union_env();
   const bool listing = union_list && dim == 2;
   int32_t* plist = listing ? nc_list : nullptr;
   int32_t* pcount = listing ? nc_list + n : nullptr;
-  if (union_nm < 0) {
-    const char* e = ab_env("RPT_UNION_NM");
-    union_nm = (e && std::atoi(e) == 0) ? 0 : 1;
-  }
   const bool nm = dim == 2 && union_pair && union_nm;
   int32_t* nm_list = nm ? cid : nullptr;
   int32_t* nm_count = nm ? cid + n : nullptr;
-  if (uf_compress < 0) {
-    const char* e = ab_env("RPT_UF_COMPRESS");
-    uf_compress = (e && std::atoi(e) == 1) ? 1 : 0;
-  }
-  cell_comp = fused && all_mutual && listing && nm && cell_comp_enabled() && !use_label_tiles() &&
-              !uf_compress;
+  cell_comp = fused && cell_comp_ok();
+  if (!cell_comp) RPT_TRY(need_float4("union_pass"));
   if (!cell_comp || !cmin_ready)
     hipLaunchKernelGGL(k_init_occ_cells, dim3(gb), dim3(kBlock), 0, st, occ, n_occ, C, rep,
                        cmin_ready ? nullptr : cmin, pcount, nm_count);
@@ -4446,9 +4594,16 @@
       if (snap)
         hipLaunchKernelGGL(k_cell_root_snapshot, dim3(grid_for(n, kBlock, 4096)), dim3(kBlock),
                            0, st, occ, n_occ, rep, parent, g.cells, uf_flags, cell_root);
-      hipLaunchKernelGGL(k_union_listed, dim3(gw), dim3(kBlock), 0, st, pts, g, occ, rec<2>(),
-                         occ_bits, slab_t, core, rep, mutual, sorig, parent, uf_flags, pm, plist,
-                         pcount, snap ? (const int32_t*)cell_root : nullptr, lstat_dev);
+      const int32_t* croot = snap ? (const int32_t*)cell_root : nullptr;
+      if (xy_points)
+        hipLaunchKernelGGL(k_union_listed<true>, dim3(gw), dim3(kBlock), 0, st,
+                           reinterpret_cast<const Pt<true>*>(pts), g, occ, rec<2>(), occ_bits,
+                           slab_t, core, rep, mutual, sorig, parent, uf_flags, pm, plist, pcount,
+                           croot, lstat_dev);
+      else
+        hipLaunchKernelGGL(k_union_listed<false>, dim3(gw), dim3(kBlock), 0, st, pts, g, occ,
+                           rec<2>(), occ_bits, slab_t, core, rep, mutual, sorig, parent, uf_flags,
+                           pm, plist, pcount, croot, lstat_dev);
     }
     else
       hipLaunchKernelGGL((k_union_cells<2, true>), dim3(gw), dim3(kBlock), 0, st, pts, g,
@@ -4486,8 +4641,8 @@
                  "[rpt stats] n=%lld occupied=%d listed_cells=%d listed: undecided=%d "
                  "roots_differ=%d searches=%d hits=%d\n",
                  (long long)n, h[0], h[1], ls[0], ls[1], ls[2], ls[3]);
-    std::fprintf(stderr, "[rpt stats] n=%lld all_mutual=%d cell_comp=%d\n", (long long)n,
-                 all_mutual ? 1 : 0, cell_comp ? 1 : 0);
+    std::fprintf(stderr, "[rpt stats] n=%lld all_mutual=%d cell_comp=%d xy_points=%d\n",
+                 (long long)n, all_mutual ? 1 : 0, cell_comp ? 1 : 0, xy_points ? 1 : 0);
   }
 #endif
   RPT_CHECK_LAUNCH();
@@ -4558,6 +4713,7 @@
       hipLaunchKernelGGL(k_label_core, dim3(glc), dim3(kBlock), 0, st, ccmin, n, sorig, mr,
                          labels);
   }
+  if (!cell_comp || label_w() != 32 || use_label_tiles()) RPT_TRY(need_float4("labels_local"));
   int32_t* kstat = nullptr;
 #ifdef RPT_AB
   if (ab_env("RPT_STATS")) {
@@ -4584,7 +4740,12 @@
                        nc_list, nc_count, labels);
   else
 #endif
-  if (cell_comp)
+  if (cell_comp && xy_points)
+    hipLaunchKernelGGL((k_label<2, false, 32, true, true>), dim3(wave_grid(n)), dim3(kBlock), 0,
+                       st, reinterpret_cast<const Pt<true>*>(pts), skey, g, rec<2>(), occ_bits,
+                       slab_t, (const int32_t*)nullptr, cell_min, mutual, sorig, mr, nc_list,
+                       nc_count, labels, kstat, core);
+  else if (cell_comp)
     hipLaunchKernelGGL((k_label<2, false, 32, true>), dim3(wave_grid(n)), dim3(kBlock), 0, st,
                        pts, skey, g, rec<2>(), occ_bits, slab_t, (const int32_t*)nullptr,
                        cell_min, mutual, sorig, mr, nc_list, nc_count, labels, kstat, core);
@@ -4652,6 +4813,7 @@
     set_error("rpt_dbscan_labels_global: degenerate parameters are handled by rpt_stdbscan");
     return RPT_ENOTSUP;
   }
+  RPT_TRY(need_float4("labels_global"));
   const int gb = grid_for(n, kBlock, 2048);
   int32_t* nc_count = nc_list + n;
   const bool cr = cell_roots_enabled();
@@ -4702,6 +4864,7 @@
 
 int32_t DbscanState::frames_pass(int32_t min_frames, hipStream_t st) {
   if (degenerate || min_frames < 1) return RPT_OK;
+  RPT_TRY(need_float4("frames_pass"));
   cmin_ready = false;
   const bool refine = min_frames >= 2;
   int32_t* list = nc_list;
@@ -4742,6 +4905,7 @@
 }
 
 int32_t DbscanState::labels_fifo(int32_t* labels, rpt_stdbscan_stats* stats, hipStream_t st) {
+  RPT_TRY(need_float4("labels_fifo"));
   int32_t* nc_count = nc_list + n;
   int32_t* spos = slab;
   RPT_TRY(cluster_ids(st, nullptr, nc_count));
@@ -4810,6 +4974,7 @@
       g_states.push_back({{dev, st}, S});
     }
   }
+  S->may_xy = stats != nullptr;
   RPT_TRY(S->build(x, y, z, stride, t, n, eps_space, eps_time, min_samples,
                    stats && stats->timing, st));
   RPT_TRY(S->core_pass(st));
@@ -4916,6 +5081,7 @@
     }
   }
   S->given_bounds = host_bounds;
+  S->may_xy = true;
   const int32_t sb = S->build(x, y, z, stride, t, n, eps_space, eps_time, min_samples,
                               stats->timing != 0, st);
   S->given_bounds = nullptr;
```

New measurement: 8012, median of 6. +4.4%, better.
